# benbergner/ips

Hardware: AMD Instinct MI355X
Metric: patches scored/sec (no-grad IPS loop) (higher is better)
Workload: dtype f32; 1 GPU; Megapixel-MNIST 1500: 2500 patches of 1x32x32 per image (BASELINE configs[1]), B=16, M=64, I=64, n_token=4, use_pos, eager; parallelism=single GPU, dedup_blank=False, patch_storage=f32, loop_workgroups_per_image=1

## Files before the change

### include/ipsx.h

```cpp
#ifndef IPSX_H
#define IPSX_H

#include <stddef.h>
#include <stdint.h>

#ifdef __cplusplus
extern "C" {
#endif

#define IPSX_VERSION 306

#define IPSX_OK            0
#define IPSX_EINVAL       -1
#define IPSX_EHIP         -2
#define IPSX_EWORKSPACE   -3

int ipsx_version(void);
const char* ipsx_last_error(void);
int ipsx_device_count(void);
int ipsx_device_is_gfx950(int dev);


size_t ipsx_packed_conv_weight_elems(int c_out, int c_in, int kh, int kw);

// ... 187 lines not shown
size_t ipsx_projector_stream_ctl_zero_words(int64_t n);
int ipsx_projector_stream_supported(const ipsx_conv* lin, int64_t n, int r);
int ipsx_projector_stats_indexed(const void* x, int dtype, const int32_t* index, int64_t src_rows, int64_t n, int f,
                                 float ln_eps, float* stats, void* stream);
int ipsx_projector_apply_indexed(const ipsx_conv* lin, const float* x, const int32_t* index, int64_t src_rows, int64_t n,
                                 const float* stats, float* out, int32_t* ready, int32_t value, void* stream);
int ipsx_projector_apply_bf16_indexed(const ipsx_conv* lin, const void* x, int dtype, const int32_t* index, int64_t src_rows,
                                      int64_t n, const float* stats, float* out, int32_t* ready, int32_t ready_value,
                                      void* stream);
int ipsx_projector_stream_indexed(const ipsx_conv* lin, const float* x, const int32_t* index, int64_t src_rows, int64_t n,
                                  int64_t slide_rows, float ln_eps, float* emb, const float* v_packed, int r, float* logits,
                                  int32_t* ctl, int32_t* ready, int workgroups, int short_first, void* stream);
int ipsx_projector_stream(const ipsx_conv* lin, const float* x, int64_t n, int64_t slide_rows, float ln_eps, float* emb,
                          const float* v_packed, int r, float* logits, int32_t* ctl, int32_t* ready,
                          int workgroups, int short_first, void* stream);


int ipsx_query_proj(const float* q, const float* wq, float temperature,
                    int n_token, int d, int hdk, float* qs, void* stream);

size_t ipsx_folded_query_elems(int h, int n_token, int d);
int ipsx_fold_query(const float* qs, const float* wk_packed, int h, int dk, int n_token, int d,
                    float* v_packed, void* stream);
int ipsx_logits(const float* emb, int64_t emb_bstride,
                const float* pos, int64_t pos_bstride,
                const float* v_packed,
                int b, int64_t n, int d, int r,
                float* logits, int64_t logits_bstride, void* stream);

int ipsx_logits_if(const float* emb, int64_t emb_bstride, const float* pos, int64_t pos_bstride,
                   const float* v_packed, int b, int64_t n, int d, int r,
                   float* logits, int64_t logits_bstride, const int32_t* cond, int32_t cond_mask, void* stream);

size_t ipsx_folded_query_bf16_bytes(int h, int n_token, int d);
int ipsx_fold_query_bf16(const float* qs, const float* wk_packed, int h, int dk, int n_token, int d,
                         void* v_packed_bf16, void* stream);
int ipsx_logits_bf16(const float* emb, int64_t emb_bstride, const float* pos, int64_t pos_bstride,
                     const void* v_packed_bf16, int b, int64_t n, int d, int r,
                     float* logits, int64_t logits_bstride, void* stream);

int ipsx_set_tie_order(int mode);

int ipsx_scan(const float* logits, int b, int64_t n, int m, int i, int h, int n_token,
              int64_t* mem_idx, float* mem_score, int32_t* tie_flag,
              void* workspace, size_t workspace_bytes, void* stream);

size_t ipsx_scan_workspace_bytes(int b, int m, int i, int h, int n_token);
int ipsx_scan_workgroups_per_image(int b, int m, int i, int h, int n_token);

int ipsx_scan_range(const float* logits, int b, int64_t n, int m, int i, int h, int n_token,
                    int64_t it_begin, int64_t it_end, int64_t* mem_idx, float* mem_score,
                    int32_t* tie_flag, void* workspace, size_t workspace_bytes, void* stream);
int ipsx_scan_range_strided(const float* logits, int64_t logits_bstride_rows, int b, int64_t n, int m, int i, int h,
                            int n_token, int64_t it_begin, int64_t it_end, int64_t* mem_idx, float* mem_score,
                            int32_t* tie_flag, void* workspace, size_t workspace_bytes, void* stream);
int ipsx_scan_ragged(const float* logits, const int64_t* row_offsets, int b, int64_t n_max, int64_t total, int m, int i,
                     int h, int n_token, int64_t* mem_idx, float* mem_score, int32_t* tie_flag, void* workspace,
                     size_t workspace_bytes, void* stream);
int ipsx_scan_ragged_spans(const float* logits, const int64_t* spans, int b, int64_t n_max, int64_t rows_total, int m, int i,
                           int h, int n_token, int64_t* mem_idx, float* mem_score, int32_t* tie_flag, void* workspace,
                           size_t workspace_bytes, void* stream);

int ipsx_scan_persistent_supported(int m, int i, int h, int n_token);
int ipsx_scan_persistent(const float* logits, int b, int64_t n, int m, int i, int h, int n_token,
                         int64_t* mem_idx, float* mem_score, int32_t* tie_flag, const int32_t* ready,
                         int32_t ready_per_image, int32_t* status, void* stream);
int ipsx_scan_persistent_groupable(int m, int i, int h, int n_token);
int ipsx_scan_persistent_on(const float* logits, int b, int64_t n, int m, int i, int h, int n_token,
                            int64_t* mem_idx, float* mem_score, int32_t* tie_flag, const int32_t* ready,
                            int32_t ready_per_image, int32_t* status, int workgroups, void* stream);
int ipsx_scan_persistent_ws(const float* logits, int b, int64_t n, int m, int i, int h, int n_token,
                            int64_t* mem_idx, float* mem_score, int32_t* tie_flag, const int32_t* ready,
                            int32_t ready_per_image, int32_t* status, int workgroups, void* workspace,
                            size_t workspace_bytes, void* stream);
int ipsx_scan_range_if_ws(const float* logits, int b, int64_t n, int m, int i, int h, int n_token,
                          int64_t it_begin, int64_t it_end, int64_t* mem_idx, float* mem_score,
                          int32_t* tie_flag, const int32_t* cond, int32_t cond_mask, void* workspace,
                          size_t workspace_bytes, void* stream);
int ipsx_publish_rows(int32_t* ready, int32_t value, void* stream);
int ipsx_set_persistent_wait_ms(int ms);
int ipsx_scan_range_if(const float* logits, int b, int64_t n, int m, int i, int h, int n_token,
                       int64_t it_begin, int64_t it_end, int64_t* mem_idx, float* mem_score,
                       int32_t* tie_flag, const int32_t* cond, int32_t cond_mask, void* stream);
int ipsx_logits_stats(const float* emb, int64_t emb_bstride, const float* pos, int64_t pos_bstride,
                      const float* v_packed, int b, int64_t n, int d, int r, float* logits, int64_t logits_bstride,
                      const float* stats_x, int64_t stats_n, int stats_f, float ln_eps, float* stats_out, void* stream);
int ipsx_scan_gate(const int32_t* status, void* stream);

int ipsx_scores(const float* x, const float* wk_packed, const float* qs,
                int b, int l, int d, int h, int dk, int n_token,
                float* scores, float* attn, void* workspace, size_t workspace_bytes,
                void* stream);
size_t ipsx_scores_workspace_bytes(int b, int l, int d, int h, int n_token);

int ipsx_topm(const float* scores, int b, int l, int m, int64_t* top_idx,
              int32_t* tie_flag, void* workspace, size_t workspace_bytes, void* stream);
size_t ipsx_topm_workspace_bytes(int b, int l, int m);

int ipsx_gather_rows(const void* src, const int64_t* idx, void* dst,
                     int b, int64_t n_rows, int m, int64_t row_bytes,
                     int64_t src_bstride_rows, void* stream);

int ipsx_ips_finish(const void* patches, int64_t patch_row_bytes, int64_t patch_bstride_rows, int64_t n_rows,
                    const void* pos, int64_t pos_row_bytes, int64_t pos_bstride_rows, const int64_t* mem_idx, int b, int m,
                    void* mem_patch, void* mem_pos, int64_t* mem_idx_out, const int32_t* status, int32_t* status_host,
                    void* stream);
int ipsx_ips_finish_indexed(const void* patches, int64_t patch_row_bytes, int64_t patch_bstride_rows, int64_t n_rows,
                            const void* pos, int64_t pos_row_bytes, int64_t pos_bstride_rows, const int64_t* mem_idx,
                            const int64_t* order, int64_t order_bstride, int b, int m, void* mem_patch, void* mem_pos,
                            int64_t* mem_idx_out, const int32_t* status, int32_t* status_host, void* stream);

int ipsx_ragged_finish(const void* rows, int64_t row_bytes, int64_t total, const int64_t* row_offsets,
                       const int64_t* mem_idx, const int32_t* flat, const void* pos, int64_t pos_row_bytes, int b, int m,
                       void* mem_patch, void* mem_pos, int64_t* mem_idx_out, int64_t* rows_out, void* stream);

typedef struct ipsx_image_entry {
    int64_t elem_off;
    int64_t first;
    int32_t h, w, ny, nx;
} ipsx_image_entry;

typedef struct ipsx_ragged_view {
    int b, c, ph, pw, sh, sw;
    const ipsx_image_entry* images;
    const ipsx_image_entry* host;
} ipsx_ragged_view;

int64_t ipsx_ragged_view_fill(ipsx_image_entry* table, int b, int c, int ph, int pw, int sh, int sw, const int32_t* h,
                              const int32_t* w, const int64_t* elem_off);
int64_t ipsx_ragged_view_offset(const ipsx_image_entry* table, int b, const ipsx_ragged_view* geometry, int64_t p,
                                int64_t* pitch, int64_t* chan_pitch);
int ipsx_trunk_ragged_view_supported(const ipsx_trunk* t, const ipsx_ragged_view* view);
int ipsx_trunk_encode_ragged_view(const ipsx_trunk* t, const float* pixels, const ipsx_ragged_view* view,
                                  const int32_t* index , int64_t first, int64_t n,
                                  float* emb, void* workspace, size_t workspace_bytes, void* stream);
int ipsx_ragged_finish_view(const float* pixels, const ipsx_ragged_view* view, const int64_t* row_offsets, const int64_t* mem_idx,
                            int m, const int32_t* flat, const void* pos, int64_t pos_row_bytes, void* mem_patch, void* mem_pos,
                            int64_t* mem_idx_out, int64_t* rows_out, void* stream);

int ipsx_ragged_view_blank_flags(const float* pixels, const ipsx_ragged_view* view, const int32_t* index,
                                 int64_t first, int64_t n, int32_t* nonblank, void* stream);
size_t ipsx_trunk_ragged_view_dedup_workspace_bytes(const ipsx_trunk* t, int64_t n);
int ipsx_trunk_encode_ragged_view_dedup(const ipsx_trunk* t, const float* pixels, const ipsx_ragged_view* view,
                                        const int32_t* index , int64_t first,
                                        int64_t n, float* emb, void* workspace, size_t workspace_bytes, int32_t* n_encoded,
                                        void* stream);

int ipsx_trunk_encode_ragged_view_u8(const ipsx_trunk* t, const uint8_t* pixels, const float* table, const ipsx_ragged_view* view,
                                     const int32_t* index , int64_t first, int64_t n,
                                     float* emb, void* workspace, size_t workspace_bytes, void* stream);
int ipsx_ragged_finish_view_u8(const uint8_t* pixels, const float* table, const ipsx_ragged_view* view, const int64_t* row_offsets,
                               const int64_t* mem_idx, int m, const int32_t* flat, const void* pos, int64_t pos_row_bytes,
                               void* mem_patch, void* mem_pos, int64_t* mem_idx_out, int64_t* rows_out, void* stream);
int ipsx_ragged_view_blank_flags_u8(const uint8_t* pixels, const ipsx_ragged_view* view, const int32_t* index, int64_t first,
                                    int64_t n, int32_t* nonblank, void* stream);
int ipsx_trunk_encode_ragged_view_dedup_u8(const ipsx_trunk* t, const uint8_t* pixels, const float* table,
                                           const ipsx_ragged_view* view, const int32_t* index, int64_t first, int64_t n, float* emb,
                                           void* workspace, size_t workspace_bytes, int32_t* n_encoded, void* stream);

typedef struct ipsx_stream_table {
    const void* held;
    int64_t held_rows, held_bstride_rows;
    const void* piece;
    int64_t piece_bstride_bytes;
    void* dst;
    int64_t dst_rows, dst_bstride_rows;
// ... 91 lines not shown
```

### ips_amd/architecture/ips_net.py

```python

import contextlib
import os

import torch
from torch import nn

from .. import hip
from ..ragged import Ragged
from ..ragged_image import RaggedImages
from ..shuffle import draw_shuffle, shuffle_batch, shuffle_instance
from .resnet import load_torchvision_checkpoint, resnet18_trunk, resnet50_trunk
from .transformer import Transformer, pos_enc_1d


class IPSNet(nn.Module):

    def get_conv_patch_enc(self, enc_type, pretrained, n_chan_in, n_res_blocks):
        if enc_type == 'resnet18':
            trunk = resnet18_trunk()
        elif enc_type == 'resnet50':
            trunk = resnet50_trunk()
        else:
            raise ValueError("unknown enc_type {!r}".format(enc_type))
        if pretrained:
# ... 156 lines not shown
            if fused:
                preds[task['name']] = hip.head(embeddings, task['id'], layer[0], task['act_fn'])
            else:
                preds[task['name']] = layer(embeddings[:, task['id']])
        return preds

    def _embed(self, x):
        if hip.on_device(x) and not self.encoder.training and not (
                torch.is_grad_enabled() and any(p.requires_grad for p in self.encoder.parameters())):
            return self.plan.encode(x, table=self._table_for(x))
        if x.dtype == torch.uint8:
            x = self._dequant(x)
        if hip.on_device(x) and self.encoder.training and self.is_image and torch.is_grad_enabled():
            from ..training import fused_encoder
            if getattr(self, "_fused_train_ok", None) is None:
                self._fused_train_ok = fused_encoder.supported(self.encoder)
            if self._fused_train_ok and fused_encoder.enabled():
                return fused_encoder.encode(self.encoder, x)
        if hip.on_device(x) and self.encoder.training and not self.is_image and torch.is_grad_enabled():
            from ..training import fused_projector
            if getattr(self, "_fused_train_ok", None) is None:
                self._fused_train_ok = fused_projector.supported(self.encoder)
            if self._fused_train_ok and fused_projector.enabled() and x.dim() == 2 and x.shape[0] > 1 and not x.requires_grad:
                return fused_projector.encode(self.encoder, x)
        if not self.is_image and x.dtype in (torch.float16, torch.bfloat16):
            x = x.float()
        return self.encoder(x).flatten(1)

    @torch.no_grad()
    def ips(self, patches):
        if isinstance(patches, Ragged):
            return self.ips_ragged(patches, pad=patches.pad)
        B, N = patches.shape[:2]
        u8 = patches.dtype == torch.uint8
        if u8:
            self._check_u8(patches)
        if self.M >= N:
            self._reset_last()
            mem_patch = patches.to(self.device)
            return (self._dequant(mem_patch) if u8 else mem_patch), (self.pos_enc.expand(B, -1, -1) if self.use_pos else None)
        return self._call(patches)

    @torch.no_grad()
    def ips_ragged(self, slides, pad=False):
        from ..ragged import ips_ragged
        return ips_ragged(self, slides, pad)

    def _reset_last(self):
        self.last_mem_idx = None
        self.last_shuffle = None
        self._emb_parts = None
        self._mem_emb = None
        self._emb_make = None
        self._mem_count = None

    @contextlib.contextmanager
    def _scoring(self):
        was_training = self.training
        if was_training:
            self.encoder.eval()
            self.transf.eval()
        try:
            yield
        finally:
            if was_training:
                self.encoder.train()
                self.transf.train()

    def _call(self, patches):
        device, pos_enc = self.device, self.pos_enc
        viewed = not torch.is_tensor(patches)
        u8 = patches.dtype == torch.uint8
        B = patches.shape[0]
        self._reset_last()
        with self._scoring():
            if self.use_pos:
                pos_enc = pos_enc.expand(B, -1, -1)
            order = None
            if self.shuffle:
                patches, pos_enc, order = self._shuffle(patches, pos_enc)

            if hip.on_device(device):
                with self.plan.hold():
                    mem_idx = self._select_hip(patches, pos_enc, order)
            else:
                mem_idx = self._select_aten(patches, pos_enc)

            src = self._device_patches if self._device_patches is not None else patches
            self._device_patches = None
            sel = self._selection
            done = sel.finish(src, pos_enc if self.use_pos else None, order) if sel is not None else None
            if done is not None:
                mem_idx, mem_patch, mem_pos = done
            else:
                if sel is not None:
                    mem_idx = sel.take_unfinished(mem_idx)
                rows = mem_idx if order is None else torch.gather(order.expand(B, -1), 1, mem_idx)
                if viewed:
                    mem_patch = hip.gather_patches_view(src.images, src.view, rows, self._table_for(src))
                else:
                    mem_patch = self._take(src, rows).to(device)
                mem_pos = self._take(pos_enc, mem_idx) if self.use_pos else None
                if sel is not None:
                    sel.after_call()
            if u8 and not viewed:
                mem_patch = self._dequant(mem_patch)

        self.last_mem_idx = mem_idx
        return mem_patch, mem_pos

    @staticmethod
    def _unfold_images(images, patch_size, patch_stride):
        (ph, pw), (sh, sw) = patch_size, patch_stride
        if ph > images.shape[2] or pw > images.shape[3] or min(ph, pw, sh, sw) <= 0:
            raise ValueError("patch {}x{} / stride {}x{} does not fit a {}x{} image".format(ph, pw, sh, sw, *images.shape[2:]))
        p = images.unfold(2, ph, sh).unfold(3, pw, sw).permute(0, 2, 3, 1, 4, 5)
        return p.reshape(images.shape[0], -1, images.shape[1], ph, pw)

    def _materialise(self, images, patch_size, patch_stride):
        if hip.on_device(self.device):
            images = images.to(self.device)
            if images.dtype == torch.float32:
                return hip.patchify(images, patch_size, patch_stride)
        return self._unfold_images(images, patch_size, patch_stride).contiguous()

    @torch.no_grad()
    def ips_image(self, images, patch_size, patch_stride):
        if isinstance(images, RaggedImages):
            return self.ips_image_ragged(images, patch_size, patch_stride, pad=images.pad)
        if not self.is_image or images.dim() != 4:
            raise TypeError("ips_image takes (B, C, H, W) images of an image encoder")
        table = self._table_for(images)
        view = None
        if (hip.on_device(self.device) and images.dtype in (torch.float32, torch.uint8) and not hip.dedup_blank()
                and not (self.encoder.training and not self.training)
                and not (self.shuffle and self._shuffle_overridden())):
            view = hip.PatchView(images.shape, patch_size, patch_stride)
            if self.M >= view.per_image or not self.plan.view_supported(view):
                view = None
        if view is None:
            return self.ips(self._materialise(images, patch_size, patch_stride))
        return self._call(hip.PatchSource(images=images.to(self.device), view=view, table=table))

    @torch.no_grad()
    def ips_image_ragged(self, images, patch_size, patch_stride, pad=False):
        from ..ragged_image import ips_image_ragged
        return ips_image_ragged(self, images, patch_size, patch_stride, pad)

    def ips_stream(self, patch_size=None, patch_stride=None):
        from ..stream import IPSStream
        return IPSStream(self, patch_size, patch_stride)

    def ips_ragged_stream(self, pad=False, patch_size=None, patch_stride=None):
        from ..ragged_stream import RaggedIPSStream
        return RaggedIPSStream(self, pad, patch_size, patch_stride)

    def _chunks(self, N):
        yield 0, self.M
        for start in range(self.M, N, self.I):
            yield start, min(start + self.I, N)

    @staticmethod
    def _take(src, idx):
        if hip.on_device(src):
            return hip.gather_rows(src, idx)
        idx = idx.to(src.device)
        view = idx.view(*idx.shape, *(1,) * (src.dim() - 2)).expand(-1, -1, *src.shape[2:])
# ... 67 lines not shown
```

### ips_amd/csrc/logits.hip

```cpp

#include <algorithm>
#include <cstdlib>

#include "scan_common.h"

namespace ipsx {

__global__ void query_proj_kernel(const float* __restrict__ q, const float* __restrict__ wq, float temperature,
                                  int n_token, int d, int hdk, float* __restrict__ qs) {
    const int i = blockIdx.x * blockDim.x + threadIdx.x;
    if (i >= n_token * hdk) return;
    const int t = i / hdk, o = i - t * hdk;
    float a = 0.0f;
    for (int c = 0; c < d; ++c) a = __builtin_fmaf(q[t * d + c], wq[(size_t)o * d + c], a);
    qs[i] = a / temperature;
}

__global__ void fold_query_kernel(const float* __restrict__ qs, const float* __restrict__ wkp, int h, int dk, int T, int d,
                                  int kgs, int r_pad, float* __restrict__ vp) {
    const int idx = blockIdx.x * blockDim.x + threadIdx.x;
    const int dpad = kgs * 8;
    if (idx >= r_pad * dpad) return;
    const int r = idx / dpad, c = idx - r * dpad;
    const int R = h * T, hdk = h * dk;
    float acc = 0.0f;
    if (r < R && c < d) {
        const int hh = r / T, t = r - hh * T;
        const int kg = c >> 3, sub = c & 7;
        for (int j = 0; j < dk; ++j) {
            const int o = hh * dk + j;
            const float w = wkp[(((size_t)(o >> 5) * kgs + kg) * 64 + (o & 31) + 32 * (sub >> 2)) * 4 + (sub & 3)];
            acc = __builtin_fmaf(qs[(size_t)t * hdk + o], w, acc);
        }
    }
    vp[(((size_t)(r >> 5) * kgs + (c >> 3)) * 64 + (r & 31) + 32 * ((c & 7) >> 2)) * 4 + (c & 3)] = acc;
}

struct LogitsArgs {
    const float* emb; long long emb_bs;
    const float* pos; long long pos_bs;
    const float* vp;
    long long n;
    int d, R, kgs;
    float* out; long long out_bs;
};

template <int NT>
__device__ __forceinline__ void logits_wave(const LogitsArgs& a, unsigned bx, int bi) {
    const int lane = threadIdx.x & 63, wave = threadIdx.x >> 6, half = lane >> 5;
    const long long r0 = ((long long)bx * 4 + wave) * 32;
    if (r0 >= a.n) return;
    const long long row = r0 + (lane & 31);
    const bool rv = row < a.n;
    const float* e = a.emb + (size_t)bi * a.emb_bs + (size_t)(rv ? row : 0) * a.d + 4 * half;
    const float* p = a.pos ? a.pos + (size_t)bi * a.pos_bs + (size_t)(rv ? row : 0) * a.d + 4 * half : nullptr;

    f32x16 acc[NT];
#pragma unroll
    for (int i = 0; i < NT; ++i)
#pragma unroll
        for (int r = 0; r < 16; ++r) acc[i][r] = 0.0f;

    const float4* vq = reinterpret_cast<const float4*>(a.vp) + lane;
    const bool vec = (a.d & 7) == 0;
    int kg0 = 0;
    if (vec) {
        float4 ev[2][8], bv[2][NT][8];
        auto fetch = [&](int k0, int set) {
#pragma unroll
            for (int u = 0; u < 8; ++u) {
                ev[set][u] = *reinterpret_cast<const float4*>(e + (k0 + u) * 8);
                if (p) {
                    const float4 pv = *reinterpret_cast<const float4*>(p + (k0 + u) * 8);
                    ev[set][u].x = ev[set][u].x + pv.x; ev[set][u].y = ev[set][u].y + pv.y;
                    ev[set][u].z = ev[set][u].z + pv.z; ev[set][u].w = ev[set][u].w + pv.w;
                }
#pragma unroll
                for (int i = 0; i < NT; ++i) bv[set][i][u] = vq[((size_t)i * a.kgs + k0 + u) * 64];
            }
        };
        auto mma = [&](int set) {
#pragma unroll
            for (int u = 0; u < 8; ++u) {
                const float a0 = rv ? ev[set][u].x : 0.0f, a1 = rv ? ev[set][u].y : 0.0f;
                const float a2 = rv ? ev[set][u].z : 0.0f, a3 = rv ? ev[set][u].w : 0.0f;
#pragma unroll
                for (int i = 0; i < NT; ++i) {
                    acc[i] = __builtin_amdgcn_mfma_f32_32x32x2f32(a0, bv[set][i][u].x, acc[i], 0, 0, 0);
                    acc[i] = __builtin_amdgcn_mfma_f32_32x32x2f32(a1, bv[set][i][u].y, acc[i], 0, 0, 0);
                    acc[i] = __builtin_amdgcn_mfma_f32_32x32x2f32(a2, bv[set][i][u].z, acc[i], 0, 0, 0);
                    acc[i] = __builtin_amdgcn_mfma_f32_32x32x2f32(a3, bv[set][i][u].w, acc[i], 0, 0, 0);
                }
            }
        };
        if (a.kgs >= 8) {
            fetch(0, 0);
            for (; kg0 + 16 <= a.kgs; kg0 += 16) {
                fetch(kg0 + 8, 1);
                mma(0);
                if (kg0 + 24 <= a.kgs) fetch(kg0 + 16, 0);
                mma(1);
            }
            if (kg0 + 8 <= a.kgs) { mma(0); kg0 += 8; }
        }
    }
    for (int kg = kg0; kg < a.kgs; ++kg) {
        float av[4];
        if (vec) {
            const float4 ev = *reinterpret_cast<const float4*>(e + kg * 8);
            av[0] = ev.x; av[1] = ev.y; av[2] = ev.z; av[3] = ev.w;
            if (p) {
                const float4 pv = *reinterpret_cast<const float4*>(p + kg * 8);
                av[0] = av[0] + pv.x; av[1] = av[1] + pv.y; av[2] = av[2] + pv.z; av[3] = av[3] + pv.w;
            }
#pragma unroll
            for (int j = 0; j < 4; ++j) av[j] = rv ? av[j] : 0.0f;
        } else {
#pragma unroll
            for (int j = 0; j < 4; ++j) {
                const int c = kg * 8 + j;
                float v = (c + 4 * half < a.d) ? e[c] : 0.0f;
                if (p) v = v + ((c + 4 * half < a.d) ? p[c] : 0.0f);
                av[j] = rv ? v : 0.0f;
            }
        }
#pragma unroll
        for (int i = 0; i < NT; ++i) {
            const float4 b = vq[((size_t)i * a.kgs + kg) * 64];
            acc[i] = __builtin_amdgcn_mfma_f32_32x32x2f32(av[0], b.x, acc[i], 0, 0, 0);
            acc[i] = __builtin_amdgcn_mfma_f32_32x32x2f32(av[1], b.y, acc[i], 0, 0, 0);
            acc[i] = __builtin_amdgcn_mfma_f32_32x32x2f32(av[2], b.z, acc[i], 0, 0, 0);
            acc[i] = __builtin_amdgcn_mfma_f32_32x32x2f32(av[3], b.w, acc[i], 0, 0, 0);
        }
    }
    float* out = a.out + (size_t)bi * a.out_bs;
#pragma unroll
    for (int i = 0; i < NT; ++i) {
        const int o = i * 32 + (lane & 31);
        if (o < a.R) {
#pragma unroll
            for (int r = 0; r < 16; ++r) {
                const long long rr = r0 + (r & 3) + 8 * (r >> 2) + 4 * half;
                if (rr < a.n) out[(size_t)rr * a.R + o] = acc[i][r];
            }
        }
    }
}

template <int NT>
__global__ __launch_bounds__(256) void logits_kernel(LogitsArgs a) { logits_wave<NT>(a, blockIdx.x, (int)blockIdx.y); }

template <int NT>
__global__ __launch_bounds__(256) void logits_if_kernel(LogitsArgs a, const int* cond, int mask) {
    if ((__hip_atomic_load(cond, __ATOMIC_RELAXED, __HIP_MEMORY_SCOPE_AGENT) & mask) == 0) return;
    logits_wave<NT>(a, blockIdx.x, (int)blockIdx.y);
}

template <int NT>
__global__ __launch_bounds__(256) void logits_stats_kernel(LogitsArgs a, unsigned n_logits_x, const float* __restrict__ sx,
                                                           long long sn, int sf, float eps, float2* __restrict__ sout) {
    if (blockIdx.x < n_logits_x) { logits_wave<NT>(a, blockIdx.x, (int)blockIdx.y); return; }
    if (blockIdx.y != 0) return;
    const int lane = threadIdx.x & 63;
    const long long row0 = ((long long)(blockIdx.x - n_logits_x) * 4 + (threadIdx.x >> 6)) * 32;
    if (row0 >= sn) return;
    const float2 st = row_moments_wave32(sx, row0, sn, sf, eps, lane);
    if (lane < 32 && row0 + lane < sn) sout[row0 + lane] = st;
}

typedef __bf16 bf16x8_t __attribute__((ext_vector_type(8)));

__global__ void fold_query_bf16_kernel(const float* __restrict__ qs, const float* __restrict__ wkp, int h, int dk, int T, int d,
                                       int kgs, int ksteps, int r_pad, unsigned short* __restrict__ vq16) {
    const int idx = blockIdx.x * blockDim.x + threadIdx.x;
    const int dpad = ksteps * 16;
    if (idx >= r_pad * dpad) return;
    const int r = idx / dpad, c = idx - r * dpad;
    const int R = h * T, hdk = h * dk;
    float acc = 0.0f;
    if (r < R && c < d) {
        const int hh = r / T, t = r - hh * T;
        const int kg = c >> 3, sub = c & 7;
        for (int j = 0; j < dk; ++j) {
            const int o = hh * dk + j;
            const float w = wkp[(((size_t)(o >> 5) * kgs + kg) * 64 + (o & 31) + 32 * (sub >> 2)) * 4 + (sub & 3)];
            acc = __builtin_fmaf(qs[(size_t)t * hdk + o], w, acc);
        }
    }
    const __bf16 hv = (__bf16)acc;
    vq16[(((size_t)(r >> 5) * ksteps + (c >> 4)) * 64 + (r & 31) + 32 * ((c & 15) >> 3)) * 8 + (c & 7)] =
        __builtin_bit_cast(unsigned short, hv);
}

template <int NT>
__global__ __launch_bounds__(256) void logits_bf16_kernel(LogitsArgs a, const uint4* __restrict__ vq16, int ksteps) {
    const int lane = threadIdx.x & 63, wave = threadIdx.x >> 6, half = lane >> 5;
    const long long r0 = ((long long)blockIdx.x * 4 + wave) * 32;
    if (r0 >= a.n) return;
    const int bi = blockIdx.y;
    const long long row = r0 + (lane & 31);
    const bool rv = row < a.n;
    const float* e = a.emb + (size_t)bi * a.emb_bs + (size_t)(rv ? row : 0) * a.d + 8 * half;
    const float* p = a.pos ? a.pos + (size_t)bi * a.pos_bs + (size_t)(rv ? row : 0) * a.d + 8 * half : nullptr;
    f32x16 acc[NT];
#pragma unroll
    for (int i = 0; i < NT; ++i)
#pragma unroll
        for (int r = 0; r < 16; ++r) acc[i][r] = 0.0f;
    for (int ks = 0; ks < ksteps; ++ks) {
        float xv[8];
#pragma unroll
        for (int j = 0; j < 8; ++j) {
            const int c = ks * 16 + 8 * half + j;
            float v = (rv && c < a.d) ? e[ks * 16 + j] : 0.0f;
            if (p) v = v + ((rv && c < a.d) ? p[ks * 16 + j] : 0.0f);
            xv[j] = v;
        }
        bf16x8_t av;
#pragma unroll
        for (int j = 0; j < 8; ++j) av[j] = (__bf16)xv[j];
#pragma unroll
        for (int i = 0; i < NT; ++i) {
            const uint4 b = vq16[((size_t)i * ksteps + ks) * 64 + lane];
            acc[i] = __builtin_amdgcn_mfma_f32_32x32x16_bf16(av, __builtin_bit_cast(bf16x8_t, b), acc[i], 0, 0, 0);
        }
    }
    float* out = a.out + (size_t)bi * a.out_bs;
#pragma unroll
    for (int i = 0; i < NT; ++i) {
// ... 147 lines not shown
```

### ips_amd/csrc/scan_common.h

```cpp
#pragma once

#include <algorithm>
#include <cstdlib>
#include <type_traits>

#include "ipsx_common.h"
#include "ipsx_math.h"
#include "ipsx_rowstats.h"
#include "ipsx_stdorder.h"

namespace ipsx {

typedef float f32x16 __attribute__((ext_vector_type(16)));

struct CandView {
    const float* cl;
    const float* lg;
    const int* cand;
    int R;
    __device__ __forceinline__ float get(int l, int r) const {
        if (cl) return cl[l * (R + 1) + r];
        const size_t row = cand ? (size_t)cand[l] : (size_t)l;
        return lg[row * R + r];
    }
// ... 822 lines not shown
                while (v_ >= 0 && v_ < (need)) {                                                               \
                    __builtin_amdgcn_s_sleep(16);                                                              \
                    int w_ = lane < a.ready_words ? __hip_atomic_load(a.ready + lane, __ATOMIC_RELAXED, __HIP_MEMORY_SCOPE_AGENT) : 0; \
                    for (int o_ = 32; o_ >= 1; o_ >>= 1) w_ += __shfl_xor(w_, o_, 64);                         \
                    const unsigned long long now_ = __builtin_amdgcn_s_memrealtime();                          \
                    if (w_ != seen_) { seen_ = w_; t0_ = now_; }                                               \
                    if (now_ - t0_ > a.wait_ticks) { v_ = -1; break; }                                         \
                    v_ = __hip_atomic_load(a.ready + b * a.ready_stride, __ATOMIC_RELAXED, __HIP_MEMORY_SCOPE_AGENT); \
                }                                                                                              \
                if (lane == 0) ccount[6] = v_;                                                     \
            }                                                                                                  \
            lds_barrier();                                                                                     \
             \
             \
            __builtin_amdgcn_fence(__ATOMIC_ACQUIRE, "agent");                                                 \
            ready_known = ccount[6];                                                               \
            if (ready_known < 0) {                                                                             \
                if (tid == 0) { __hip_atomic_fetch_or(a.status, 1, __ATOMIC_RELAXED, __HIP_MEMORY_SCOPE_AGENT); a.plog[5] += 1; } \
                return;                                                                                        \
            }                                                                                                  \
        }                                                                                                      \
    } while (0)

template <int N, int J>
__device__ __forceinline__ uint32_t cmpx32(uint32_t s, uint32_t dir, int lane) {
    const uint32_t o = lane_xor_u32<J>(s, lane);
    const uint32_t c = (uint32_t)__builtin_amdgcn_sbfe((int)dir, N, 1);
    uint32_t d;
    asm("v_med3_u32 %0, %1, %2, %3" : "=v"(d) : "v"(s), "v"(o), "v"(c));
    return d;
}

__device__ __forceinline__ uint32_t sort_directions(int lane) {
    constexpr int KJ[21][2] = {{2, 1}, {4, 2}, {4, 1}, {8, 4}, {8, 2}, {8, 1}, {16, 8}, {16, 4}, {16, 2}, {16, 1}, {32, 16}, {32, 8},
                               {32, 4}, {32, 2}, {32, 1}, {64, 32}, {64, 16}, {64, 8}, {64, 4}, {64, 2}, {64, 1}};
    uint32_t d = 0u;
#pragma unroll
    for (int n = 0; n < 21; ++n) d |= ((((lane & KJ[n][0]) == 0) == ((lane & KJ[n][1]) == 0)) ? 1u : 0u) << n;
    return d;
}

__device__ __forceinline__ uint32_t wave_sort_desc_u32(uint32_t s, uint32_t dir, int lane) {
    s = cmpx32<0, 1>(s, dir, lane);
    s = cmpx32<1, 2>(s, dir, lane); s = cmpx32<2, 1>(s, dir, lane);
    s = cmpx32<3, 4>(s, dir, lane); s = cmpx32<4, 2>(s, dir, lane); s = cmpx32<5, 1>(s, dir, lane);
    s = cmpx32<6, 8>(s, dir, lane); s = cmpx32<7, 4>(s, dir, lane); s = cmpx32<8, 2>(s, dir, lane); s = cmpx32<9, 1>(s, dir, lane);
    s = cmpx32<10, 16>(s, dir, lane); s = cmpx32<11, 8>(s, dir, lane); s = cmpx32<12, 4>(s, dir, lane); s = cmpx32<13, 2>(s, dir, lane);
    s = cmpx32<14, 1>(s, dir, lane);
    s = cmpx32<15, 32>(s, dir, lane); s = cmpx32<16, 16>(s, dir, lane); s = cmpx32<17, 8>(s, dir, lane); s = cmpx32<18, 4>(s, dir, lane);
    s = cmpx32<19, 2>(s, dir, lane); s = cmpx32<20, 1>(s, dir, lane);
    return s;
}

struct TopmArgs {
    int tie_order, stk_off;
    const float* scores;
    int L, m, n2;
    long long* top;
    int* tie;
};

struct ScanCall {
    const float* logits = nullptr;
    int b = 0;
    int64_t n = 0;
    int m = 0, i = 0, h = 0, n_token = 0;
    int64_t it_begin = 0, it_end = 0;
    int64_t* mem_idx = nullptr;
    float* mem_score = nullptr;
    int32_t* tie_flag = nullptr;
    const int32_t* ready = nullptr;
    int32_t* status = nullptr;
    void* workspace = nullptr;
    size_t workspace_bytes = 0;
    void* stream = nullptr;
    const int32_t* cond = nullptr;
    int32_t cond_mask = 0;
    int ready_stride = 0, workgroups = 0;
    Rows rows = Rows::Packed;
    const int64_t* slide_table = nullptr;
    int64_t table_rows = 0;
};

inline const long long* slide_entries(const ScanCall& c) {
    static_assert(sizeof(long long) == sizeof(int64_t), "slide tables: 64-bit entries");
    return static_cast<const long long*>(static_cast<const void*>(c.slide_table));
}

struct FastPlan {
    bool ok;
    int ept, lch;
    size_t lds;
};
FastPlan scan_fast_plan(int m, int i, int h, int n_token);
int launch_scan_fast(const ScanCall& c, const FastPlan& fp);
bool scan_cam_shape(int m, int i, int h, int n_token);
int launch_scan_cam(const ScanCall& c);
bool scan_mnist_shape(int m, int i, int h, int n_token);
int launch_scan_mnist(const ScanCall& c);
size_t scan_large_ws_per_image(int m, int i, int h, int n_token);
int launch_scan_large(const ScanCall& c);
int scan_large_team(int b, int m, int i, int h, int n_token);
int launch_topm_large(const TopmArgs& a, int b, void* workspace, size_t workspace_bytes, void* stream);
size_t topm_large_ws_per_row(int l);
int scan_large_max_l();

extern int g_persist_wait_ms;
extern bool g_scan_generic;
extern bool g_replay_stamps_on;
extern bool g_scan_direct;
extern bool g_scan_team_trunc;
extern int g_scan_team;
extern bool g_scan_r8;
extern bool g_scan_mnist;
extern unsigned long long* g_scan_stamps;
unsigned long long* persist_log();

inline int next_pow2(int v) { int p = 1; while (p < v) p <<= 1; return p; }
constexpr size_t kLdsLimit = 160 * 1024;

inline void fill_scan_args(ScanArgs& a, const ScanCall& c) {
    a.plog = persist_log();
    a.lg = c.logits; a.n = c.n; a.table_rows = c.table_rows; a.m = c.m; a.i = c.i; a.h = c.h; a.T = c.n_token; a.n2 = next_pow2(c.m + c.i);
    a.it0 = c.it_begin; a.it1 = c.it_end;
    a.mem_idx = reinterpret_cast<long long*>(c.mem_idx); a.mem_score = c.mem_score; a.tie = c.tie_flag;
    a.ready = c.ready; a.status = c.status; a.ready_stride = c.ready_stride;
    a.ready_words = c.ready ? (c.ready_stride ? std::min(c.b, 64) : 1) : 0;
    a.wait_ticks = (unsigned long long)g_persist_wait_ms * 100000ull;
    a.cond = c.cond; a.cond_mask = c.cond_mask;
    a.slides = c.b;
    a.tie_order = g_tie_order;
    a.use_lds = 1;
    a.stk_off = 0;
}

template <typename T> struct as_declared { using type = T; };
template <typename... A>
inline void launch_lds(void (*kernel)(A...), dim3 grid, dim3 block, size_t lds, void* stream, typename as_declared<A>::type... args) {
    (void)hipFuncSetAttribute(reinterpret_cast<const void*>(kernel), hipFuncAttributeMaxDynamicSharedMemorySize, (int)lds);
    kernel<<<grid, block, lds, as_stream(stream)>>>(args...);
}

}
```

### ips_amd/csrc/scan_mnist.hip

```cpp

#include <algorithm>
#include <cstdlib>

#include "scan_common.h"

namespace ipsx {

namespace mn {
constexpr int M = 64, I = 64, L = 128, R = 32, H = 8, T = 4, LD = 36, NT = 1024;
constexpr int OFF_KEYA = 0;
constexpr int OFF_SORTED = OFF_KEYA + L * 8;
constexpr int OFF_CAND = OFF_SORTED + L * 8;
constexpr int OFF_PMAX = OFF_CAND + 2 * L * 4;
constexpr int OFF_CNT = OFF_PMAX + 4 * R * 4;
constexpr int OFF_PREV = OFF_CNT + 32;
constexpr int OFF_DEN = OFF_PREV + 2 * R * 4;
constexpr int OFF_X = (OFF_DEN + R * 4 + 15) & ~15;
constexpr int OFF_E = OFF_X + 2 * L * LD * 4;
constexpr int OFF_STK = OFF_E + 2 * L * LD * 4;
constexpr int LDS_BYTES = OFF_STK + STK_BYTES;
static_assert(OFF_KEYA % 16 == 0 && OFF_X % 16 == 0 && (LD * 4) % 16 == 0, "16-byte rows");
static_assert(H * T == R && M + I == L && L * 8 == NT, "scan_mnist_kernel: 8 threads per key");
static_assert(OFF_STK == 77728, "scan_mnist_kernel: 77,728 B of LDS + the replay's scratch (STK_BYTES)");
static_assert(LDS_BYTES <= 160 * 1024, "scan_mnist_kernel: LDS");
}

template <int K>
__device__ __forceinline__ float quad_bcast(float v) {
    return as_float((uint32_t)__builtin_amdgcn_update_dpp(0, (int)as_u32(v), K * 0x55, 0xF, 0xF, false));
}

template <bool PERSIST>
__global__ __launch_bounds__(mn::NT) void scan_mnist_kernel(ScanArgs a) {
    using namespace mn;
    extern __shared__ __attribute__((aligned(16))) unsigned char smem[];
    if (!PERSIST && scan_skipped(a.cond, a.cond_mask)) return;
    __builtin_amdgcn_s_setprio(3);
    if (PERSIST) {
        asm volatile("v_mov_b32 v127, 0" ::: "v127");
        if (threadIdx.x == 0) {
            __hip_atomic_fetch_or(a.status, 2, __ATOMIC_RELAXED, __HIP_MEMORY_SCOPE_AGENT);
            __hip_atomic_store(&a.plog[4], (unsigned long long)__builtin_amdgcn_s_memrealtime(), __ATOMIC_RELAXED, __HIP_MEMORY_SCOPE_AGENT);
        }
    }
    uint64_t* const keyA = reinterpret_cast<uint64_t*>(smem + OFF_KEYA);
    uint64_t* const sorted = reinterpret_cast<uint64_t*>(smem + OFF_SORTED);
    uint32_t* const pmax = reinterpret_cast<uint32_t*>(smem + OFF_PMAX);
    int* const ccount = reinterpret_cast<int*>(smem + OFF_CNT);
    uint32_t* const prevk = reinterpret_cast<uint32_t*>(smem + OFF_PREV);
    float* const rden = reinterpret_cast<float*>(smem + OFF_DEN);
    const int tid = threadIdx.x, lane = tid & 63, wave = tid >> 6;
    const int b = blockIdx.x;
    const int r = tid & (R - 1);
    const int hid = tid - 512;
    const float* const lg = a.lg + (size_t)b * a.n * R;
    int ready_known = 0;
    if (tid < 4 * R) pmax[tid] = 0u;
    if (tid < 2) ccount[2 + tid] = 0;
    lds_barrier();
    SCAN_WAIT_ROWS(std::min<long long>(a.n, a.it0 * (long long)I + M + I));
    {
        float* const x0 = reinterpret_cast<float*>(smem + OFF_X);
        int* const cand0 = reinterpret_cast<int*>(smem + OFF_CAND);
        uint32_t km = 0u;
#pragma unroll
        for (int k = 0; k < 2; ++k) {
            const int l = (tid >> 5) + 32 * k;
            const size_t row = a.it0 == 0 ? (size_t)l : (size_t)a.mem_idx[(size_t)b * M + l];
            const float v = scan_load<PERSIST>(lg + row * R + r);
            x0[l * LD + r] = v;
            km = max(km, max_key(v));
        }
        fold_row_max<R>(km, pmax, lane);
        if (tid < M) cand0[tid] = a.it0 == 0 ? tid : (int)a.mem_idx[(size_t)b * M + tid];
    }
    const long long n_iter = a.it1 - a.it0;
    float pf[4];
    {
        float* const x0 = reinterpret_cast<float*>(smem + OFF_X);
        int* const cand0 = reinterpret_cast<int*>(smem + OFF_CAND);
        const long long lo = a.it0 * (long long)I + M;
        const int cnt = n_iter > 0 ? (int)std::min<long long>(I, a.n - lo) : 0;
        uint32_t kc = 0u;
#pragma unroll
        for (int k = 0; k < 2; ++k) {
            const int e = tid + NT * k;
            if (e < cnt * R) {
                const float v = scan_load<PERSIST>(lg + (size_t)lo * R + e);
                x0[(M + (e >> 5)) * LD + r] = v;
                kc = max(kc, max_key(v));
            }
        }
        fold_row_max<R>(kc, pmax + R, lane);
        if (tid < cnt) cand0[M + tid] = (int)(lo + tid);
        const long long lo1 = lo + I;
        const int cnt1 = n_iter > 1 ? (int)std::max<long long>(0, std::min<long long>(I, a.n - lo1)) : 0;
        if (cnt1 > 0) SCAN_WAIT_ROWS(lo1 + cnt1);
#pragma unroll
        for (int k = 0; k < 4; ++k) {
            const int e = hid + 512 * k;
            pf[k] = (hid >= 0 && e < cnt1 * R) ? scan_load<PERSIST>(lg + (size_t)lo1 * R + e) : 0.0f;
        }
    }
    int tie = 0;
    const int n_it = (int)n_iter, n_rows = (int)a.n;
    for (int k_it = 0; k_it < n_it; ++k_it) {
        const int lo = ((int)a.it0 + k_it) * I + M;
        const int cnt = min(I, n_rows - lo);
        const int Lc = M + cnt;
        const int par = k_it & 1;
        float* const xc = reinterpret_cast<float*>(smem + OFF_X) + par * (L * LD);
        float* const xn = reinterpret_cast<float*>(smem + OFF_X) + (par ^ 1) * (L * LD);
        float* const ec = reinterpret_cast<float*>(smem + OFF_E) + par * (L * LD);
        float* const en = reinterpret_cast<float*>(smem + OFF_E) + (par ^ 1) * (L * LD);
        int* const cand = reinterpret_cast<int*>(smem + OFF_CAND) + par * L;
        int* const cnew = reinterpret_cast<int*>(smem + OFF_CAND) + (par ^ 1) * L;
        uint32_t* const mkey = pmax + 2 * R * par;
        uint32_t* const mkey_nx = pmax + 2 * R * (par ^ 1);
        const int lo1 = lo + I;
        const int cnt1 = k_it + 1 < n_it ? max(0, min(I, n_rows - lo1)) : 0;
        lds_barrier();
        if (tid == 0) ccount[2 + (par ^ 1)] = 0;
        const uint32_t mbits = as_u32(max_key_value(max(mkey[r], mkey[R + r])));
        const float rowmax = as_float(mbits);
        const bool changed = k_it == 0 || prevk[par * R + r] != mbits;
        if (tid < R) prevk[(par ^ 1) * R + r] = mbits;
        {
            unsigned long long moved = __ballot(changed) & 0xFFFFFFFFull;
            if (moved != 0ull) {
                if (__popcll(moved) >= 8) {
                    if (changed) {
#pragma unroll
                        for (int k = 0; k < 4; ++k) {
                            const int l = (tid >> 5) + 32 * k;
                            if (l < Lc) ec[l * LD + r] = det_expf_np(xc[l * LD + r] - rowmax);
                        }
                    }
                } else {
                    while (moved) {
                        const int rr = __ffsll((long long)moved) - 1;
                        moved &= moved - 1ull;
                        exp_column(xc + rr, ec + rr, Lc, LD, __shfl(rowmax, rr, 64));
// ... 62 lines not shown
            const uint32_t* const sw = reinterpret_cast<const uint32_t*>(sorted);
            const unsigned long long eqm = __ballot(sw[2 * lane + 1] == sw[2 * lane + 3]);
            if (eqm != 0ull) {
                if (a.tie_order != 0) {
                    bool hit = false;
                    for (int j = tid; j < M && !hit; j += NT)
                        for (int k = j + 1; k < Lc && !hit && (sorted[k] >> 32) == (sorted[j] >> 32); ++k) {
                            bool same = true;
                            if (a.tie_order == 1) {
                                const uint4* ra = reinterpret_cast<const uint4*>(xc + key_pos(sorted[j]) * LD);
                                const uint4* rb = reinterpret_cast<const uint4*>(xc + key_pos(sorted[k]) * LD);
                                uint32_t diff = 0u;
#pragma unroll
                                for (int rr = 0; rr < R / 4; ++rr) {
                                    const uint4 va = ra[rr], vb = rb[rr];
                                    diff |= (va.x ^ vb.x) | (va.y ^ vb.y) | (va.z ^ vb.z) | (va.w ^ vb.w);
                                }
                                same = diff == 0u;
                            }
                            hit = hit || same;
                        }
                    if (__ballot(hit) != 0ull && lane == 0) ccount[2 + par] = 1;
                }
                lds_barrier();
                if (tid == 0 && (eqm >> (M - 1)) != 0ull) tie = 1;
                if (a.tie_order != 0 && ccount[2 + par] != 0)
                    tie_order_slow(sorted, keyA, Lc, M, reinterpret_cast<int*>(smem + OFF_STK));
            }
        }
        {
            const int lo2 = lo + 2 * I;
            const int cnt2 = k_it + 2 < n_it ? max(0, min(I, n_rows - lo2)) : 0;
            if (cnt2 > 0) SCAN_WAIT_ROWS(lo2 + cnt2);
#pragma unroll
            for (int k = 0; k < 4; ++k) {
                const int e = hid + 512 * k;
                pf[k] = (hid >= 0 && e < cnt2 * R) ? scan_load<PERSIST>(lg + (size_t)lo2 * R + e) : 0.0f;
            }
        }
        {
            const uint32_t* const spos = reinterpret_cast<const uint32_t*>(sorted);
            if (wave < 8) {
                uint32_t p[4];
#pragma unroll
                for (int k = 0; k < 4; ++k) p[k] = ~spos[2 * ((tid >> 5) + 16 * k)] & (L - 1);
                float gx[4];
#pragma unroll
                for (int k = 0; k < 4; ++k) gx[k] = xc[p[k] * LD + r];
                uint32_t km = 0u;
#pragma unroll
                for (int k = 0; k < 4; ++k) { xn[((tid >> 5) + 16 * k) * LD + r] = gx[k]; km = max(km, max_key(gx[k])); }
                fold_row_max<R>(km, mkey_nx, lane);
            } else {
                const int j = hid >> 3, qd = (hid & 7) * 4;
                const uint32_t p = ~spos[2 * j] & (L - 1);
                const uint32_t pc = ~spos[2 * (hid & (M - 1))] & (L - 1);
                const float4 ge = *reinterpret_cast<const float4*>(ec + p * LD + qd);
                const int ci = cand[pc];
                *reinterpret_cast<float4*>(en + j * LD + qd) = ge;
                if (hid < M) cnew[hid] = ci;
            }
        }
    }
    lds_barrier();
    {
        const int parn = (int)(n_iter & 1);
        const int* const cand = reinterpret_cast<const int*>(smem + OFF_CAND) + parn * L;
        if (tid < M) {
            a.mem_idx[(size_t)b * M + tid] = cand[tid];
            if (a.mem_score) a.mem_score[(size_t)b * M + tid] = n_iter > 0 ? key_score(sorted[tid]) : 0.0f;
        }
    }
    if (a.tie && tid == 0 && tie) a.tie[b] = 1;
}

bool scan_mnist_shape(int m, int i, int h, int n_token) { return h == mn::H && n_token == mn::T && m == mn::M && i == mn::I; }

int launch_scan_mnist(const ScanCall& c) {
    IPSX_REQUIRE(scan_mnist_shape(c.m, c.i, c.h, c.n_token) && c.rows == Rows::Packed && (c.workgroups <= 0 || c.workgroups >= c.b),
                 "scan_mnist_kernel: 8 heads x 4 tokens, M = I = 64, contiguous logits, one workgroup per image");
    ScanArgs a;
    fill_scan_args(a, c);
    a.stk_off = mn::OFF_STK;
    launch_lds(c.ready ? scan_mnist_kernel<true> : scan_mnist_kernel<false>, dim3((unsigned)c.b), dim3(mn::NT), mn::LDS_BYTES, c.stream, a);
    return launched("scan");
}

}
```

### ips_amd/csrc/scorer.hip

```cpp

#include <algorithm>
#include <cstdlib>

#include "scan_common.h"

namespace ipsx {

int g_tie_order = 1;
int g_persist_wait_ms = 50;
bool g_scan_generic = false;
bool g_replay_stamps_on = false;
bool g_scan_team_trunc = true;
int g_scan_team = -1;
bool g_scan_direct = true;
bool g_scan_r8 = true;
bool g_scan_mnist = true;
unsigned long long* g_scan_stamps = nullptr;

__device__ unsigned long long g_persist_log[8];


unsigned long long* persist_log() {
    static unsigned long long* p[64] = {nullptr};
    int dev = 0;
    if (hipGetDevice(&dev) != hipSuccess || dev < 0 || dev >= 64) dev = 0;
    if (!p[dev]) {
        void* q = nullptr;
        if (hipGetSymbolAddress(&q, HIP_SYMBOL(g_persist_log)) == hipSuccess) p[dev] = static_cast<unsigned long long*>(q);
    }
    return p[dev];
}

static ScanCall scan_call(const float* logits, int b, int64_t n, int m, int i, int h, int n_token, int64_t* mem_idx,
                          float* mem_score, int32_t* tie_flag, void* stream) {
    ScanCall c;
    c.logits = logits; c.b = b; c.n = n; c.m = m; c.i = i; c.h = h; c.n_token = n_token;
    c.mem_idx = mem_idx; c.mem_score = mem_score; c.tie_flag = tie_flag; c.stream = stream;
    return c;
}

static void whole_loop(ScanCall& c) { c.it_begin = 0; c.it_end = (c.n - c.m + c.i - 1) / c.i; }

static int validate_scan_call(const ScanCall& c) {
    IPSX_REQUIRE(c.logits && c.mem_idx, "scan: null pointer");
    IPSX_REQUIRE(c.b > 0 && c.m > 0 && c.i > 0 && c.h > 0 && c.n_token > 0, "scan: bad sizes");
    IPSX_REQUIRE(c.n > c.m, "scan: needs more patches (%lld) than memory slots (%d)", (long long)c.n, c.m);
    IPSX_REQUIRE(c.n < ((int64_t)1 << 31), "scan: too many patches");
    IPSX_REQUIRE(c.it_begin >= 0 && c.it_begin <= c.it_end && c.it_end <= (c.n - c.m + c.i - 1) / c.i,
                 "scan: iteration range [%lld, %lld) outside the loop", (long long)c.it_begin, (long long)c.it_end);
    if (c.rows == Rows::Packed) return IPSX_OK;
    IPSX_REQUIRE(!c.ready && !c.cond && !g_scan_stamps,
                 "scan: only packed logits are waited for (persistent), launched conditionally or stamped");
    IPSX_REQUIRE(c.table_rows > 0 && c.table_rows < ((int64_t)1 << 31), "scan: a table of %lld rows", (long long)c.table_rows);
    if (rows_per_slide(c.rows)) {
        IPSX_REQUIRE(c.slide_table, "scan: slides without their table");
        IPSX_REQUIRE(c.workgroups <= 0 || c.workgroups >= c.b, "scan: slides of different lengths take a workgroup each");
    }
    return IPSX_OK;
}

static int dispatch_scan(const ScanCall& c) {
    IPSX_TRY(validate_scan_call(c));
    if (c.it_begin == c.it_end) return IPSX_OK;
    const FastPlan fp = scan_fast_plan(c.m, c.i, c.h, c.n_token);
    if (!fp.ok || (g_scan_generic && !c.ready && !c.cond)) return launch_scan_large(c);
    if (g_scan_r8 && scan_cam_shape(c.m, c.i, c.h, c.n_token)) return launch_scan_cam(c);
    if (g_scan_mnist && scan_mnist_shape(c.m, c.i, c.h, c.n_token) && c.rows == Rows::Packed &&
        (c.workgroups <= 0 || c.workgroups >= c.b) && g_scan_stamps == nullptr)
        return launch_scan_mnist(c);
    return launch_scan_fast(c, fp);
}

}

using namespace ipsx;

IPSX_API int ipsx_scan(const float* logits, int b, int64_t n, int m, int i, int h, int n_token,
                       int64_t* mem_idx, float* mem_score, int32_t* tie_flag, void* workspace, size_t workspace_bytes,
                       void* stream) {
    IPSX_REQUIRE(n > m && i > 0, "scan: needs more patches (%lld) than memory slots (%d)", (long long)n, m);
    if (tie_flag && hipMemsetAsync(tie_flag, 0, sizeof(int32_t) * (size_t)std::max(b, 0), as_stream(stream)) != hipSuccess)
        return fail(IPSX_EHIP, "scan: memset failed");
    return ipsx_scan_range(logits, b, n, m, i, h, n_token, 0, (n - m + i - 1) / i, mem_idx, mem_score, tie_flag,
                           workspace, workspace_bytes, stream);
}

IPSX_API int ipsx_scan_range(const float* logits, int b, int64_t n, int m, int i, int h, int n_token,
                             int64_t it_begin, int64_t it_end, int64_t* mem_idx, float* mem_score,
                             int32_t* tie_flag, void* workspace, size_t workspace_bytes, void* stream) {
    ScanCall c = scan_call(logits, b, n, m, i, h, n_token, mem_idx, mem_score, tie_flag, stream);
    c.it_begin = it_begin; c.it_end = it_end;
    c.workspace = workspace; c.workspace_bytes = workspace_bytes;
    return dispatch_scan(c);
}

IPSX_API int ipsx_scan_range_strided(const float* logits, int64_t logits_bstride_rows, int b, int64_t n, int m, int i, int h,
                                     int n_token, int64_t it_begin, int64_t it_end, int64_t* mem_idx, float* mem_score,
                                     int32_t* tie_flag, void* workspace, size_t workspace_bytes, void* stream) {
    IPSX_REQUIRE(logits_bstride_rows >= n && logits_bstride_rows < ((int64_t)1 << 31),
// ... 101 lines not shown
    whole_loop(c);
    c.ready = ready; c.ready_stride = ready_per_image ? 1 : 0; c.status = status;
    c.workgroups = workgroups;
    c.workspace = workspace; c.workspace_bytes = workspace_bytes;
    return dispatch_scan(c);
}

IPSX_API int ipsx_scan_range_if_ws(const float* logits, int b, int64_t n, int m, int i, int h, int n_token,
                                   int64_t it_begin, int64_t it_end, int64_t* mem_idx, float* mem_score,
                                   int32_t* tie_flag, const int32_t* cond, int32_t cond_mask, void* workspace,
                                   size_t workspace_bytes, void* stream) {
    IPSX_REQUIRE(cond && cond_mask, "scan_range_if: needs the condition word and a mask");
    ScanCall c = scan_call(logits, b, n, m, i, h, n_token, mem_idx, mem_score, tie_flag, stream);
    c.it_begin = it_begin; c.it_end = it_end;
    c.cond = cond; c.cond_mask = cond_mask;
    c.workspace = workspace; c.workspace_bytes = workspace_bytes;
    return dispatch_scan(c);
}

__global__ void scan_gate_kernel(const int* status, unsigned long long wait_ticks) {
    const unsigned long long t0 = __builtin_amdgcn_s_memrealtime();
    bool gave_up = false;
    while ((__hip_atomic_load(status, __ATOMIC_RELAXED, __HIP_MEMORY_SCOPE_AGENT) & 2) == 0) {
        __builtin_amdgcn_s_sleep(8);
        if (__builtin_amdgcn_s_memrealtime() - t0 > wait_ticks) { gave_up = true; break; }
    }
    const unsigned long long waited = __builtin_amdgcn_s_memrealtime() - t0;
    g_persist_log[0] += 1;
    g_persist_log[3] = t0;
    if (gave_up) g_persist_log[2] += 1;
    if (waited > g_persist_log[1]) {
        g_persist_log[1] = waited;
        g_persist_log[6] = t0;
        g_persist_log[7] = gave_up ? 0ull : __hip_atomic_load(&g_persist_log[4], __ATOMIC_RELAXED, __HIP_MEMORY_SCOPE_AGENT);
    }
}

IPSX_API int ipsx_scan_gate(const int32_t* status, void* stream) {
    IPSX_REQUIRE(status, "scan_gate: null pointer");
    scan_gate_kernel<<<dim3(1), dim3(1), 0, as_stream(stream)>>>(status, (unsigned long long)g_persist_wait_ms * 100000ull);
    return launched("scan_gate");
}

__global__ void part_wait_kernel(const int* done, int want, int* status, int bit, unsigned long long wait_ticks) {
    unsigned long long t0 = __builtin_amdgcn_s_memrealtime();
    int last = __hip_atomic_load(done, __ATOMIC_RELAXED, __HIP_MEMORY_SCOPE_AGENT);
    while (last < want) {
        __builtin_amdgcn_s_sleep(32);
        const int v = __hip_atomic_load(done, __ATOMIC_RELAXED, __HIP_MEMORY_SCOPE_AGENT);
        const unsigned long long t = __builtin_amdgcn_s_memrealtime();
        if (v != last) { last = v; t0 = t; }
        else if (t - t0 > wait_ticks) {
            __hip_atomic_fetch_or(status, bit, __ATOMIC_RELAXED, __HIP_MEMORY_SCOPE_AGENT);
            break;
        }
    }
    __builtin_amdgcn_fence(__ATOMIC_ACQUIRE, "agent");
}

IPSX_API int ipsx_part_wait(const int32_t* done, int32_t want, int32_t* status, int32_t bit, void* stream) {
    IPSX_REQUIRE(done && status && bit, "part_wait: needs the counter, the status word and a bit");
    part_wait_kernel<<<dim3(1), dim3(1), 0, as_stream(stream)>>>(done, want, status, bit,
                                                                 (unsigned long long)g_persist_wait_ms * 100000ull);
    return launched("part_wait");
}

IPSX_API int ipsx_publish_rows(int32_t* ready, int32_t value, void* stream) {
    IPSX_REQUIRE(ready, "publish_rows: null pointer");
    publish_rows_kernel<<<dim3(1), dim3(1), 0, as_stream(stream)>>>(ready, value);
    return launched("publish_rows");
}

IPSX_API int ipsx_scan_range_if(const float* logits, int b, int64_t n, int m, int i, int h, int n_token,
                                int64_t it_begin, int64_t it_end, int64_t* mem_idx, float* mem_score,
                                int32_t* tie_flag, const int32_t* cond, int32_t cond_mask, void* stream) {
    IPSX_REQUIRE(cond && cond_mask, "scan_range_if: needs the condition word and a mask");
    IPSX_REQUIRE(scan_fast_plan(m, i, h, n_token).ok, "scan_range_if: shapes of the LDS-resident loop only");
    ScanCall c = scan_call(logits, b, n, m, i, h, n_token, mem_idx, mem_score, tie_flag, stream);
    c.it_begin = it_begin; c.it_end = it_end;
    c.cond = cond; c.cond_mask = cond_mask;
    return dispatch_scan(c);
}

IPSX_API int ipsx_set_persistent_wait_ms(int ms) {
    const int prev = g_persist_wait_ms;
    if (ms > 0) g_persist_wait_ms = ms > 20000 ? 20000 : ms;
    return prev;
}

IPSX_API int ipsx_set_tie_order(int mode) {
    const int prev = ipsx::g_tie_order;
    if (mode >= 0 && mode <= 2) ipsx::g_tie_order = mode;
    return prev;
}

extern "C" __attribute__((visibility("default"))) int ipsx_dbg_persist_log(unsigned long long* out8) {
    unsigned long long zero[8] = {0, 0, 0, 0, 0, 0, 0, 0};
    if (hipMemcpyFromSymbol(out8, HIP_SYMBOL(ipsx::g_persist_log), sizeof(zero)) != hipSuccess) return -1;
    return hipMemcpyToSymbol(HIP_SYMBOL(ipsx::g_persist_log), zero, sizeof(zero)) == hipSuccess ? 0 : -1;
}

extern "C" __attribute__((visibility("default"))) void ipsx_dbg_scan_stamps(unsigned long long* buf) {
    ipsx::g_scan_stamps = buf;
}

extern "C" __attribute__((visibility("default"))) void ipsx_dbg_scan_generic(int on) { g_scan_generic = on != 0; }

extern "C" __attribute__((visibility("default"))) void ipsx_dbg_scan_direct(int on) { g_scan_direct = on != 0; }
extern "C" __attribute__((visibility("default"))) void ipsx_dbg_scan_team(int w) { g_scan_team = w; }
extern "C" __attribute__((visibility("default"))) void ipsx_dbg_scan_team_trunc(int on) { g_scan_team_trunc = on != 0; }
extern "C" __attribute__((visibility("default"))) void ipsx_dbg_scan_r8(int on) { g_scan_r8 = on != 0; }
extern "C" __attribute__((visibility("default"))) void ipsx_dbg_scan_mnist(int on) { g_scan_mnist = on != 0; }
extern "C" __attribute__((visibility("default"))) int ipsx_dbg_scan_mnist_shape(int m, int i, int h, int n_token) {
    return scan_mnist_shape(m, i, h, n_token) ? 1 : 0;
}
```

### ips_amd/hip.py

```python

import collections
import ctypes as C
import os
import subprocess

import torch

_PKG = os.path.dirname(os.path.abspath(__file__))
_SO = os.path.join(_PKG, "lib", "libipsx.so")
_LIB = None

f32p = C.c_void_p
ABI_MAJOR = 3


def backend():
    b = os.environ.get("IPSX_BACKEND", "hip").lower()
    if b not in ("hip", "aten"):
        raise ValueError("IPSX_BACKEND must be 'hip' or 'aten', got {!r}".format(b))
    return b


def precision():
    p = os.environ.get("IPSX_PRECISION", "fp32").lower()
# ... 223 lines not shown
    "ipsx_projector_stats_indexed": (C.c_int, [C.c_void_p, C.c_int, C.c_void_p, C.c_int64, C.c_int64, C.c_int, C.c_float, C.c_void_p,
                                               C.c_void_p]),
    "ipsx_projector_apply_indexed": (C.c_int, [C.POINTER(Conv), C.c_void_p, C.c_void_p, C.c_int64, C.c_int64, C.c_void_p, C.c_void_p,
                                               C.c_void_p, C.c_int32, C.c_void_p]),
    "ipsx_projector_apply_bf16_indexed": (C.c_int, [C.POINTER(Conv), C.c_void_p, C.c_int, C.c_void_p, C.c_int64, C.c_int64, C.c_void_p,
                                                    C.c_void_p, C.c_void_p, C.c_int32, C.c_void_p]),
    "ipsx_projector_stream_indexed": (C.c_int, [C.POINTER(Conv), C.c_void_p, C.c_void_p, C.c_int64, C.c_int64, C.c_int64, C.c_float,
                                                C.c_void_p, C.c_void_p, C.c_int, C.c_void_p, C.c_void_p, C.c_void_p, C.c_int, C.c_int,
                                                C.c_void_p]),
    "ipsx_trunk_stream_ctl_words": (C.c_size_t, [C.c_int64]),
    "ipsx_trunk_stream_supported": (C.c_int, [C.POINTER(Trunk), C.c_int, C.c_int]),
    "ipsx_trunk_stream": (C.c_int, [C.POINTER(Trunk), C.c_void_p, C.c_int64, C.c_void_p, C.c_void_p, C.c_void_p, C.c_int,
                                    C.c_void_p, C.c_void_p, C.c_void_p, C.c_int, C.c_int, C.c_void_p]),
    "ipsx_projector_stream_ctl_words": (C.c_size_t, [C.c_int64]),
    "ipsx_projector_stream_ctl_zero_words": (C.c_size_t, [C.c_int64]),
    "ipsx_projector_stream_supported": (C.c_int, [C.POINTER(Conv), C.c_int64, C.c_int]),
    "ipsx_projector_stream": (C.c_int, [C.POINTER(Conv), C.c_void_p, C.c_int64, C.c_int64, C.c_float, C.c_void_p, C.c_void_p, C.c_int,
                                        C.c_void_p, C.c_void_p, C.c_void_p, C.c_int, C.c_int, C.c_void_p]),
    "ipsx_logits_stats": (C.c_int, [C.c_void_p, C.c_int64, C.c_void_p, C.c_int64, C.c_void_p,
                                    C.c_int, C.c_int64, C.c_int, C.c_int, C.c_void_p, C.c_int64,
                                    C.c_void_p, C.c_int64, C.c_int, C.c_float, C.c_void_p, C.c_void_p]),
    "ipsx_query_proj": (C.c_int, [C.c_void_p, C.c_void_p, C.c_float, C.c_int, C.c_int, C.c_int,
                                  C.c_void_p, C.c_void_p]),
    "ipsx_folded_query_elems": (C.c_size_t, [C.c_int, C.c_int, C.c_int]),
    "ipsx_fold_query": (C.c_int, [C.c_void_p, C.c_void_p, C.c_int, C.c_int, C.c_int, C.c_int, C.c_void_p, C.c_void_p]),
    "ipsx_logits": (C.c_int, [C.c_void_p, C.c_int64, C.c_void_p, C.c_int64, C.c_void_p,
                              C.c_int, C.c_int64, C.c_int, C.c_int,
                              C.c_void_p, C.c_int64, C.c_void_p]),
    "ipsx_folded_query_bf16_bytes": (C.c_size_t, [C.c_int, C.c_int, C.c_int]),
    "ipsx_fold_query_bf16": (C.c_int, [C.c_void_p, C.c_void_p, C.c_int, C.c_int, C.c_int, C.c_int, C.c_void_p, C.c_void_p]),
    "ipsx_logits_bf16": (C.c_int, [C.c_void_p, C.c_int64, C.c_void_p, C.c_int64, C.c_void_p,
                                   C.c_int, C.c_int64, C.c_int, C.c_int,
                                   C.c_void_p, C.c_int64, C.c_void_p]),
    "ipsx_set_tie_order": (C.c_int, [C.c_int]),
    "ipsx_scan": (C.c_int, [C.c_void_p, C.c_int, C.c_int64, C.c_int, C.c_int, C.c_int, C.c_int,
                            C.c_void_p, C.c_void_p, C.c_void_p, C.c_void_p, C.c_size_t, C.c_void_p]),
    "ipsx_scan_workspace_bytes": (C.c_size_t, [C.c_int] * 5),
    "ipsx_scan_workgroups_per_image": (C.c_int, [C.c_int] * 5),
    "ipsx_scan_range": (C.c_int, [C.c_void_p, C.c_int, C.c_int64, C.c_int, C.c_int, C.c_int, C.c_int, C.c_int64, C.c_int64,
                                  C.c_void_p, C.c_void_p, C.c_void_p, C.c_void_p, C.c_size_t, C.c_void_p]),
    "ipsx_scan_range_strided": (C.c_int, [C.c_void_p, C.c_int64, C.c_int, C.c_int64, C.c_int, C.c_int, C.c_int, C.c_int, C.c_int64,
                                          C.c_int64, C.c_void_p, C.c_void_p, C.c_void_p, C.c_void_p, C.c_size_t, C.c_void_p]),
    "ipsx_scan_ragged": (C.c_int, [C.c_void_p, C.c_void_p, C.c_int, C.c_int64, C.c_int64, C.c_int, C.c_int, C.c_int, C.c_int,
                                   C.c_void_p, C.c_void_p, C.c_void_p, C.c_void_p, C.c_size_t, C.c_void_p]),
    "ipsx_stream_commit": (C.c_int, [C.POINTER(StreamTable), C.c_int, C.c_void_p, C.c_int, C.c_int, C.c_int64, C.c_int64,
                                     C.c_void_p]),
    "ipsx_stream_commit_view": (C.c_int, [C.POINTER(StreamTable), C.c_int, C.c_void_p, C.POINTER(PatchViewStruct), C.c_int,
                                          C.c_void_p, C.c_int, C.c_int, C.c_int64, C.c_int64, C.POINTER(C.c_int), C.c_void_p]),
    "ipsx_scan_range_if": (C.c_int, [C.c_void_p, C.c_int, C.c_int64, C.c_int, C.c_int, C.c_int, C.c_int, C.c_int64, C.c_int64,
                                     C.c_void_p, C.c_void_p, C.c_void_p, C.c_void_p, C.c_int32, C.c_void_p]),
    "ipsx_scan_persistent_supported": (C.c_int, [C.c_int] * 4),
    "ipsx_scan_persistent_groupable": (C.c_int, [C.c_int] * 4),
    "ipsx_scan_persistent_on": (C.c_int, [C.c_void_p, C.c_int, C.c_int64, C.c_int, C.c_int, C.c_int, C.c_int,
                                          C.c_void_p, C.c_void_p, C.c_void_p, C.c_void_p, C.c_int32, C.c_void_p, C.c_int,
                                          C.c_void_p]),
    "ipsx_scan_persistent_ws": (C.c_int, [C.c_void_p, C.c_int, C.c_int64, C.c_int, C.c_int, C.c_int, C.c_int,
                                          C.c_void_p, C.c_void_p, C.c_void_p, C.c_void_p, C.c_int32, C.c_void_p, C.c_int,
                                          C.c_void_p, C.c_size_t, C.c_void_p]),
    "ipsx_scan_range_if_ws": (C.c_int, [C.c_void_p, C.c_int, C.c_int64, C.c_int, C.c_int, C.c_int, C.c_int, C.c_int64, C.c_int64,
                                        C.c_void_p, C.c_void_p, C.c_void_p, C.c_void_p, C.c_int32, C.c_void_p, C.c_size_t,
                                        C.c_void_p]),
    "ipsx_scan_persistent": (C.c_int, [C.c_void_p, C.c_int, C.c_int64, C.c_int, C.c_int, C.c_int, C.c_int,
                                       C.c_void_p, C.c_void_p, C.c_void_p, C.c_void_p, C.c_int32, C.c_void_p, C.c_void_p]),
    "ipsx_publish_rows": (C.c_int, [C.c_void_p, C.c_int32, C.c_void_p]),
    "ipsx_set_persistent_wait_ms": (C.c_int, [C.c_int]),
    "ipsx_scan_gate": (C.c_int, [C.c_void_p, C.c_void_p]),
    "ipsx_trunk_encode_indexed": (C.c_int, [C.POINTER(Trunk), C.c_void_p, C.c_void_p, C.c_int64, C.c_void_p, C.c_void_p]),
    "ipsx_trunk_encode_parts": (C.c_int, [C.POINTER(Trunk), C.c_void_p, C.c_void_p, C.c_int64, C.c_void_p,
                                          C.POINTER(C.c_int64), C.c_int, C.c_void_p, C.c_void_p]),
    "ipsx_trunk_parts_dedup_workspace_bytes": (C.c_size_t, [C.POINTER(Trunk), C.c_int64]),
    "ipsx_trunk_encode_parts_dedup": (C.c_int, [C.POINTER(Trunk), C.c_void_p, C.c_void_p, C.c_int64, C.c_void_p,
                                                C.POINTER(C.c_int64), C.c_int, C.c_void_p, C.c_void_p, C.c_void_p, C.c_size_t,
                                                C.c_void_p, C.c_void_p]),
    "ipsx_trunk_encode_parts_dedup_u8": (C.c_int, [C.POINTER(Trunk), C.c_void_p, C.c_void_p, C.c_void_p, C.c_int64, C.c_void_p,
                                                   C.POINTER(C.c_int64), C.c_int, C.c_void_p, C.c_void_p, C.c_void_p, C.c_size_t,
                                                   C.c_void_p, C.c_void_p]),
    "ipsx_trunk_encode_parts_dedup_view": (C.c_int, [C.POINTER(Trunk), C.c_void_p, C.POINTER(PatchViewStruct), C.c_void_p, C.c_int64,
                                                     C.c_void_p, C.POINTER(C.c_int64), C.c_int, C.c_void_p, C.c_void_p, C.c_void_p,
                                                     C.c_size_t, C.c_void_p, C.c_void_p]),
    "ipsx_trunk_encode_parts_dedup_view_u8": (C.c_int, [C.POINTER(Trunk), C.c_void_p, C.c_void_p, C.POINTER(PatchViewStruct),
                                                        C.c_void_p, C.c_int64, C.c_void_p, C.POINTER(C.c_int64), C.c_int, C.c_void_p,
                                                        C.c_void_p, C.c_void_p, C.c_size_t, C.c_void_p, C.c_void_p]),
    "ipsx_part_wait": (C.c_int, [C.c_void_p, C.c_int32, C.c_void_p, C.c_int32, C.c_void_p]),
    "ipsx_logits_if": (C.c_int, [C.c_void_p, C.c_int64, C.c_void_p, C.c_int64, C.c_void_p, C.c_int, C.c_int64, C.c_int, C.c_int,
                                 C.c_void_p, C.c_int64, C.c_void_p, C.c_int32, C.c_void_p]),
    "ipsx_trunk_encode_u8": (C.c_int, [C.POINTER(Trunk), C.c_void_p, C.c_void_p, C.c_int64, C.c_void_p, C.c_void_p,
                                       C.c_size_t, C.c_void_p]),
    "ipsx_trunk_encode_indexed_u8": (C.c_int, [C.POINTER(Trunk), C.c_void_p, C.c_void_p, C.c_void_p, C.c_int64, C.c_void_p,
                                               C.c_void_p]),
    "ipsx_dequant_patches": (C.c_int, [C.c_void_p, C.c_void_p, C.c_void_p, C.c_int64, C.c_int, C.c_int, C.c_void_p]),
    "ipsx_scores_workspace_bytes": (C.c_size_t, [C.c_int] * 5),
    "ipsx_scores": (C.c_int, [C.c_void_p, C.c_void_p, C.c_void_p] + [C.c_int] * 6 +
                    [C.c_void_p, C.c_void_p, C.c_void_p, C.c_size_t, C.c_void_p]),
    "ipsx_topm": (C.c_int, [C.c_void_p, C.c_int, C.c_int, C.c_int, C.c_void_p, C.c_void_p, C.c_void_p, C.c_size_t, C.c_void_p]),
    "ipsx_topm_workspace_bytes": (C.c_size_t, [C.c_int] * 3),
    "ipsx_gather_rows": (C.c_int, [C.c_void_p, C.c_void_p, C.c_void_p, C.c_int, C.c_int64, C.c_int,
                                   C.c_int64, C.c_int64, C.c_void_p]),
    "ipsx_ips_call_run": (C.c_int, [C.POINTER(IpsCall)]),
    "ipsx_ips_call_elapsed": (C.c_int, [C.c_int, C.POINTER(C.c_float)]),
    "ipsx_ips_call_run_ordered": (C.c_int, [C.POINTER(IpsCall), C.POINTER(IpsCallOrder)]),
    "ipsx_order_index": (C.c_int, [C.c_void_p, C.c_int64, C.c_int, C.c_int64, C.c_void_p, C.c_void_p]),
    "ipsx_trunk_stream_indexed": (C.c_int, [C.POINTER(Trunk), C.c_void_p, C.c_void_p, C.c_int64, C.c_int64, C.c_void_p, C.c_void_p,
                                            C.c_void_p, C.c_int, C.c_void_p, C.c_void_p, C.c_void_p, C.c_int, C.c_int, C.c_void_p]),
    "ipsx_ips_finish": (C.c_int, [C.c_void_p, C.c_int64, C.c_int64, C.c_int64, C.c_void_p, C.c_int64, C.c_int64, C.c_void_p, C.c_int,
                                  C.c_int, C.c_void_p, C.c_void_p, C.c_void_p, C.c_void_p, C.c_void_p, C.c_void_p]),
    "ipsx_ips_finish_indexed": (C.c_int, [C.c_void_p, C.c_int64, C.c_int64, C.c_int64, C.c_void_p, C.c_int64, C.c_int64, C.c_void_p,
                                          C.c_void_p, C.c_int64, C.c_int, C.c_int, C.c_void_p, C.c_void_p, C.c_void_p, C.c_void_p,
                                          C.c_void_p, C.c_void_p]),
    "ipsx_ragged_finish": (C.c_int, [C.c_void_p, C.c_int64, C.c_int64, C.c_void_p, C.c_void_p, C.c_void_p, C.c_void_p, C.c_int64,
                                     C.c_int, C.c_int, C.c_void_p, C.c_void_p, C.c_void_p, C.c_void_p, C.c_void_p]),
    "ipsx_ragged_view_fill": (C.c_int64, [C.POINTER(ImageEntry)] + [C.c_int] * 6 + [C.POINTER(C.c_int32), C.POINTER(C.c_int32),
                                          C.POINTER(C.c_int64)]),
    "ipsx_ragged_view_offset": (C.c_int64, [C.POINTER(ImageEntry), C.c_int, C.POINTER(RaggedViewStruct), C.c_int64,
                                            C.POINTER(C.c_int64), C.POINTER(C.c_int64)]),
    "ipsx_trunk_ragged_view_supported": (C.c_int, [C.POINTER(Trunk), C.POINTER(RaggedViewStruct)]),
    "ipsx_trunk_encode_ragged_view": (C.c_int, [C.POINTER(Trunk), C.c_void_p, C.POINTER(RaggedViewStruct), C.c_void_p, C.c_int64,
                                                C.c_int64, C.c_void_p, C.c_void_p, C.c_size_t, C.c_void_p]),
    "ipsx_ragged_finish_view": (C.c_int, [C.c_void_p, C.POINTER(RaggedViewStruct), C.c_void_p, C.c_void_p, C.c_int, C.c_void_p,
                                          C.c_void_p, C.c_int64, C.c_void_p, C.c_void_p, C.c_void_p, C.c_void_p, C.c_void_p]),
    "ipsx_ragged_view_blank_flags": (C.c_int, [C.c_void_p, C.POINTER(RaggedViewStruct), C.c_void_p, C.c_int64, C.c_int64, C.c_void_p,
                                               C.c_void_p]),
    "ipsx_trunk_ragged_view_dedup_workspace_bytes": (C.c_size_t, [C.POINTER(Trunk), C.c_int64]),
    "ipsx_trunk_encode_ragged_view_dedup": (C.c_int, [C.POINTER(Trunk), C.c_void_p, C.POINTER(RaggedViewStruct), C.c_void_p, C.c_int64,
                                                      C.c_int64, C.c_void_p, C.c_void_p, C.c_size_t, C.c_void_p, C.c_void_p]),
    "ipsx_trunk_encode_ragged_view_u8": (C.c_int, [C.POINTER(Trunk), C.c_void_p, C.c_void_p, C.POINTER(RaggedViewStruct), C.c_void_p,
                                                   C.c_int64, C.c_int64, C.c_void_p, C.c_void_p, C.c_size_t, C.c_void_p]),
    "ipsx_ragged_finish_view_u8": (C.c_int, [C.c_void_p, C.c_void_p, C.POINTER(RaggedViewStruct), C.c_void_p, C.c_void_p, C.c_int,
                                             C.c_void_p, C.c_void_p, C.c_int64, C.c_void_p, C.c_void_p, C.c_void_p, C.c_void_p,
                                             C.c_void_p]),
    "ipsx_ragged_view_blank_flags_u8": (C.c_int, [C.c_void_p, C.POINTER(RaggedViewStruct), C.c_void_p, C.c_int64, C.c_int64,
                                                  C.c_void_p, C.c_void_p]),
    "ipsx_trunk_encode_ragged_view_dedup_u8": (C.c_int, [C.POINTER(Trunk), C.c_void_p, C.c_void_p, C.POINTER(RaggedViewStruct),
                                                         C.c_void_p, C.c_int64, C.c_int64, C.c_void_p, C.c_void_p, C.c_size_t,
                                                         C.c_void_p, C.c_void_p]),
    "ipsx_scan_ragged_spans": (C.c_int, [C.c_void_p, C.c_void_p, C.c_int, C.c_int64, C.c_int64, C.c_int, C.c_int, C.c_int, C.c_int,
                                         C.c_void_p, C.c_void_p, C.c_void_p, C.c_void_p, C.c_size_t, C.c_void_p]),
    "ipsx_stream_commit_ragged": (C.c_int, [C.POINTER(StreamTable), C.c_int, C.c_void_p, C.c_void_p, C.c_int, C.c_int, C.c_int64,
                                            C.c_int64, C.c_void_p]),
    "ipsx_stream_commit_ragged_view": (C.c_int, [C.POINTER(StreamTable), C.c_int, C.c_void_p, C.POINTER(RaggedViewStruct), C.c_int,
                                                 C.c_void_p, C.c_void_p, C.c_int, C.c_int, C.c_int64, C.c_int64, C.POINTER(C.c_int),
                                                 C.c_void_p]),
    "ipsx_aggregate_workspace_bytes": (C.c_size_t, [C.POINTER(Transf), C.c_int, C.c_int]),
    "ipsx_aggregate": (C.c_int, [C.POINTER(Transf), C.c_void_p, C.c_int, C.c_int, C.c_void_p,
                                 C.c_void_p, C.c_size_t, C.c_void_p]),
    "ipsx_aggregate_packed": (C.c_int, [C.POINTER(Transf), C.c_void_p, C.c_void_p, C.c_void_p, C.c_int, C.c_int, C.c_void_p,
                                        C.c_void_p, C.c_size_t, C.c_void_p]),
    "ipsx_head": (C.c_int, [C.c_void_p, C.c_int, C.c_int, C.c_int, C.c_int, C.c_void_p, C.c_void_p,
                            C.c_int, C.c_int, C.c_void_p, C.c_void_p]),
    "ipsx_bn_train_supported": (C.c_int, [C.c_int64, C.c_int]),
    "ipsx_bn_train_workspace_floats": (C.c_size_t, [C.c_int64, C.c_int]),
    "ipsx_bn_train_forward": (C.c_int, [C.c_void_p, C.c_void_p, C.c_int64, C.c_int, C.c_void_p, C.c_void_p,
                                        C.c_float, C.c_float, C.c_void_p, C.c_void_p, C.c_int,
                                        C.c_void_p, C.c_void_p, C.c_void_p, C.c_void_p, C.c_void_p]),
    "ipsx_bn_train_backward": (C.c_int, [C.c_void_p, C.c_void_p, C.c_void_p, C.c_int64, C.c_int, C.c_void_p,
                                         C.c_void_p, C.c_void_p, C.c_int, C.c_void_p, C.c_void_p, C.c_void_p,
                                         C.c_void_p, C.c_void_p, C.c_void_p]),
    "ipsx_projector_train_supported": (C.c_int, [C.c_int, C.c_int]),
    "ipsx_projector_train_slabs": (C.c_int64, [C.c_int64]),
    "ipsx_projector_train_forward": (C.c_int, [C.POINTER(Conv), C.c_void_p, C.c_void_p, C.c_int, C.c_int64, C.c_void_p, C.c_void_p,
                                               C.c_void_p, C.c_void_p, C.c_void_p]),
    "ipsx_projector_wgrad_chunk_rows": (C.c_int64, []),
    "ipsx_projector_wgrad_max_rows": (C.c_int64, [C.c_int, C.c_int, C.c_int]),
    "ipsx_projector_wgrad_workspace_bytes": (C.c_size_t, [C.c_int64, C.c_int, C.c_int]),
    "ipsx_projector_wgrad": (C.c_int, [C.c_void_p, C.c_int, C.c_void_p, C.c_void_p, C.c_int64, C.c_int, C.c_int, C.c_void_p,
                                       C.c_void_p, C.c_int, C.c_void_p, C.c_size_t, C.c_void_p]),
    "ipsx_attn_pool_supported": (C.c_int, [C.c_int, C.c_int]),
    "ipsx_attn_pool_workspace_bytes": (C.c_size_t, [C.c_int64, C.c_int64, C.c_int, C.c_int]),
    "ipsx_attn_pool_forward": (C.c_int, [C.c_void_p, C.c_void_p, C.c_void_p, C.c_int64, C.c_int64, C.c_int, C.c_int, C.c_void_p,
                                         C.c_void_p, C.c_void_p, C.c_size_t, C.c_void_p]),
    "ipsx_attn_pool_backward": (C.c_int, [C.c_void_p, C.c_void_p, C.c_void_p, C.c_void_p, C.c_void_p, C.c_void_p, C.c_int64,
                                          C.c_int64, C.c_int, C.c_int, C.c_void_p, C.c_void_p, C.c_void_p, C.c_size_t, C.c_void_p]),
}


def library_path():
    return _SO


def build(verbose=False):
    cmd = ["make", "-C", os.path.join(_PKG, "csrc")] + ([] if verbose else ["-s"])
    subprocess.check_call(cmd)
    return _SO


def lib():
    global _LIB
    if _LIB is None:
        if not os.path.exists(_SO):
            raise RuntimeError(
                "libipsx.so not found at {} - build it with `python -c 'import __graft_entry__ as g; "
                "g.build()'` or `make -C ips_amd/csrc`; the HIP backend has no fallback".format(_SO))
        L = C.CDLL(_SO)
        for name, (res, args) in _EXPORTS.items():
            fn = getattr(L, name)
            fn.restype, fn.argtypes = res, args
        if L.ipsx_version() // 100 != ABI_MAJOR:
            raise RuntimeError("libipsx.so ABI version {} != {}.x (include/ipsx.h: the major number changes with every "
                               "incompatible change of an exported signature)".format(L.ipsx_version(), ABI_MAJOR))
        L.ipsx_set_tie_order(_TIE_MODES[tie_order()])
        if os.environ.get("IPSX_CAM_HEAD"):
            L.ipsx_dbg_stream_head.restype, L.ipsx_dbg_stream_head.argtypes = None, [C.c_int]
            L.ipsx_dbg_stream_head(int(os.environ["IPSX_CAM_HEAD"]))
        if os.environ.get("IPSX_SCAN_R8", "1") == "0":
            L.ipsx_dbg_scan_r8.argtypes = [C.c_int]
            L.ipsx_dbg_scan_r8(0)
        _LIB = L
    return _LIB


def _ck(rc, what):
    if rc != 0:
        raise RuntimeError("{} failed ({}): {}".format(what, rc, lib().ipsx_last_error().decode()))


def _stream():
    return C.c_void_p(_raw_stream(_cur_device()))


_raw_stream = getattr(torch._C, "_cuda_getCurrentRawStream", None)
_cur_device = getattr(torch._C, "_cuda_getDevice", None)
if _raw_stream is None or _cur_device is None:
    def _stream():
        return C.c_void_p(torch.cuda.current_stream().cuda_stream)


def _p(t):
    return C.c_void_p(t.data_ptr()) if t is not None else C.c_void_p(0)


def _f32(t):
    if t.dtype != torch.float32:
        raise TypeError("expected float32, got {}".format(t.dtype))
    return t if t.is_contiguous() else t.contiguous()


def _same_gpu(what, names, *tensors):
    dev = None
    for t in tensors:
        if t is not None:
            d = t.device
            if dev is None:
                if not _gpu_device(d):
                    raise ValueError("{}: {} lies on {}, the kernels read and write GPU memory".format(
                        what, [n for n, u in zip(names, tensors) if u is t][0], d))
                dev = d
            elif d != dev:
                raise ValueError("{}: {} lies on {}, the call's other tensors on {}".format(
                    what, [n for n, u in zip(names, tensors) if u is t][0], d, dev))
    return dev


def _one_gpu(what, **tensors):
    return _same_gpu(what, tuple(tensors), *tensors.values())


def _rd(what, name, t, dtype=torch.float32, dim=None, align=16, cl=False):
    if t.dtype != dtype:
        raise TypeError("{}: {} must be {}, got {}".format(what, name, dtype, t.dtype))
    if dim is not None and t.dim() != dim:
        raise ValueError("{}: {} must have {} dimensions, got {}".format(what, name, dim, tuple(t.shape)))
    if cl:
        if not t.is_contiguous(memory_format=torch.channels_last):
            return t.contiguous(memory_format=torch.channels_last)
    elif not t.is_contiguous():
        return t.contiguous()
    return t.clone() if t.data_ptr() % align else t


def _wr(what, name, t, dtype, shape=None, align=1, cl=False):
    if t.dtype != dtype or (shape is not None and tuple(t.shape) != tuple(shape)) or t.data_ptr() % align or \
            not (t.is_contiguous(memory_format=torch.channels_last) if cl else t.is_contiguous()):
        raise ValueError("{}: {} must be a {}{} {} tensor{}, got {} {} with strides {} at an address {} mod 16".format(
            what, name, "channels-last" if cl else "contiguous", " " + str(tuple(shape)) if shape is not None else "", dtype,
            " at a {}-byte address".format(align) if align > 1 else "", t.dtype, tuple(t.shape), t.stride(), t.data_ptr() % 16))
    return t


def _workspace(what, ws):
    return _wr(what, "workspace", ws, torch.uint8, align=16) if ws is not None else None


_PATCH_DTYPES = {torch.float32: 0, torch.bfloat16: 1, torch.float16: 2}


def _patch_table(table, n_chan, device):
    from .quant import check_table
    check_table(table, n_chan)
    if table.device != device:
# ... 141 lines not shown
def _word(what, name, t, n=1):
    if t.dtype != torch.int32 or t.numel() != n or not t.is_contiguous():
        raise ValueError("{}: {} must hold {} contiguous int32 word(s), got {} {}".format(what, name, n, t.dtype, tuple(t.shape)))
    return t


def part_wait(done, want, status, bit=1):
    _same_gpu("part_wait", ("done", "status"), done, status)
    _word("part_wait", "done", done)
    _word("part_wait", "status", status)
    _ck(lib().ipsx_part_wait(_p(done), int(want), _p(status), int(bit), _stream()), "ipsx_part_wait")


def logits_stats(emb, pos, vq, R, out, stats_x, stats_out, ln_eps):
    _same_gpu("logits_stats", ("emb", "stats_x", "stats_out"), emb, stats_x, stats_out)
    if vq.dtype != torch.float32:
        raise TypeError("logits_stats: vq must be the float32 folded query, got {}".format(vq.dtype))
    if out is None:
        raise ValueError("logits_stats: out must be given")
    stats_x = _rd("logits_stats", "stats_x", stats_x, dim=2)
    sn, sf = stats_x.shape
    _wr("logits_stats", "stats_out", stats_out, torch.float32, (sn, 2), align=8)
    emb, pos, pos_bs, out = _logits_args("logits_stats", emb, pos, vq, R, out, None)
    B, n, D = emb.shape
    _ck(lib().ipsx_logits_stats(_p(emb), n * D, _p(pos), pos_bs, _p(vq), B, n, D, R, _p(out), out.stride(0),
                                _p(stats_x), sn, sf, C.c_float(ln_eps), _p(stats_out), _stream()), "ipsx_logits_stats")
    return out


def scan_workspace(B, M, I, H, T, device):
    nb = lib().ipsx_scan_workspace_bytes(B, M, I, H, T)
    return torch.empty(nb, dtype=torch.uint8, device=device) if nb else None


def scan_workgroups_per_image(B, M, I, H, T):
    return max(1, int(lib().ipsx_scan_workgroups_per_image(B, M, I, H, T)))


def _scan_args(what, lg, M, I, H, T, mem_idx=None, tie=None, workspace=None, copy=True, words=()):
    _same_gpu(what, _SCAN_NAMES, lg, mem_idx, tie, workspace, *words)
    shape = lg.shape
    if len(shape) != 3 or shape[2] != H * T:
        raise ValueError("{}: lg must be (B, N, H*T = {}), got {}".format(what, H * T, tuple(shape)))
    B, N = shape[0], shape[1]
    if N <= M:
        raise ValueError("{}: lg has N = {} rows per image, the loop needs more than M = {}".format(what, N, M))
    if lg.dtype != torch.float32:
        raise TypeError("{}: lg must be float32, got {}".format(what, lg.dtype))
    if not lg.is_contiguous() or lg.data_ptr() & 15:
        if not copy:
            raise ValueError("{}: lg must be the whole contiguous (B, N, H*T) table at a 16-byte address (it is read where it "
                             "lies), got strides {}".format(what, lg.stride()))
        lg = lg.clone() if lg.is_contiguous() else lg.contiguous()
    if mem_idx is not None and (mem_idx.dtype != torch.int64 or mem_idx.shape != (B, M) or not mem_idx.is_contiguous()):
        raise ValueError("{}: mem_idx must be a contiguous ({}, {}) int64 tensor, got {} {}".format(what, B, M, mem_idx.dtype, tuple(mem_idx.shape)))
    if tie is not None and (tie.dtype != torch.int32 or tie.shape != (B,) or not tie.is_contiguous()):
        raise ValueError("{}: tie must be a contiguous ({},) int32 tensor, got {} {}".format(what, B, tie.dtype, tuple(tie.shape)))
    if workspace is not None:
        _workspace(what, workspace)
    return lg, B, N


_SCAN_NAMES = ("lg", "mem_idx", "tie", "workspace", "cond / ready", "status")


def scan(lg, M, I, H, T, want_scores=False):
    lg, B, N = _scan_args("scan", lg, M, I, H, T)
    mem_idx = torch.empty((B, M), dtype=torch.int64, device=lg.device)
    sc = torch.empty((B, M), dtype=torch.float32, device=lg.device) if want_scores else None
    tie = torch.zeros((B,), dtype=torch.int32, device=lg.device)
    ws = scan_workspace(B, M, I, H, T, lg.device)
    _ck(lib().ipsx_scan(_p(lg), B, N, M, I, H, T, _p(mem_idx), _p(sc), _p(tie), _p(ws), ws.numel() if ws is not None else 0,
                        _stream()), "ipsx_scan")
    scan.last_tie = tie
    return (mem_idx, sc) if want_scores else mem_idx


def scan_range(lg, M, I, H, T, it_begin, it_end, mem_idx, tie, workspace=None):
    lg, B, N = _scan_args("scan_range", lg, M, I, H, T, mem_idx, tie, workspace)
    ws = workspace if workspace is not None else scan_workspace(B, M, I, H, T, lg.device)
    _ck(lib().ipsx_scan_range(_p(lg), B, N, M, I, H, T, it_begin, it_end, _p(mem_idx), None, _p(tie),
                              _p(ws), ws.numel() if ws is not None else 0, _stream()), "ipsx_scan_range")
    return mem_idx


def scan_range_strided(lg, n, M, I, H, T, it_begin, it_end, mem_idx, tie, workspace=None):
    B, cap = lg.shape[:2]
    if lg.dtype != torch.float32 or lg.dim() != 3 or lg.stride(2) != 1 or lg.stride(1) != lg.shape[2] or (B > 1 and lg.stride(0) != cap * lg.shape[2]):
        raise ValueError("scan_range_strided needs a row-contiguous float32 (B, cap, H*T) logits table")
    if lg.shape[2] != H * T or lg.data_ptr() % 16:
        raise ValueError("scan_range_strided: lg must have H*T = {} columns and lie at a 16-byte address, got {}".format(H * T, tuple(lg.shape)))
    if not 0 < n <= cap:
        raise ValueError("{} candidates in a table of {} rows".format(n, cap))
    _one_gpu("scan_range_strided", lg=lg, mem_idx=mem_idx, tie=tie, workspace=workspace)
    _wr("scan_range_strided", "mem_idx", mem_idx, torch.int64, (B, M))
    _wr("scan_range_strided", "tie", tie, torch.int32, (B,))
    _workspace("scan_range_strided", workspace)
    ws = workspace if workspace is not None else scan_workspace(B, M, I, H, T, lg.device)
    _ck(lib().ipsx_scan_range_strided(_p(lg), cap, B, n, M, I, H, T, it_begin, it_end, _p(mem_idx), None, _p(tie),
                                      _p(ws), ws.numel() if ws is not None else 0, _stream()), "ipsx_scan_range_strided")
    return mem_idx


def scan_ragged(lg, offsets, lengths, M, I, H, T, want_scores=False, workspace=None, short_ok=False):
    lengths = [int(n) for n in lengths]
    B, total = len(lengths), sum(lengths)
    if B == 0:
        raise ValueError("scan_ragged: no slides")
    _one_gpu("scan_ragged", lg=lg, offsets=offsets, workspace=workspace)
    _workspace("scan_ragged", workspace)
    if lg.data_ptr() % 16:
        raise ValueError("scan_ragged: lg must lie at a 16-byte address")
    if lg.dtype != torch.float32 or lg.dim() != 2 or not lg.is_contiguous() or lg.shape != (total, H * T):
        raise ValueError("scan_ragged needs a contiguous float32 ({}, {}) logits table, got {} {}".format(
            total, H * T, lg.dtype, tuple(lg.shape)))
    if offsets.dtype != torch.int64 or tuple(offsets.shape) != (B + 1,) or not offsets.is_contiguous() or offsets.device != lg.device:
        raise ValueError("scan_ragged needs the ({},) int64 row offsets on the logits' device".format(B + 1))
    for k, n in enumerate(lengths):
        if n <= M and not short_ok:
            raise ValueError("slide {} has {} rows: the loop needs more than M = {}".format(k, n, M))
    if max(lengths) <= M:
        raise ValueError("scan_ragged: no slide has more than M = {} rows".format(M))
    mem_idx = torch.empty((B, M), dtype=torch.int64, device=lg.device)
    sc = torch.empty((B, M), dtype=torch.float32, device=lg.device) if want_scores else None
    tie = torch.empty((B,), dtype=torch.int32, device=lg.device)
    ws = workspace
    if ws is None:
        nb = lib().ipsx_scan_workspace_bytes(1, M, I, H, T)
        ws = torch.empty(B * nb, dtype=torch.uint8, device=lg.device) if nb else None
    _ck(lib().ipsx_scan_ragged(_p(lg), _p(offsets), B, max(lengths), total, M, I, H, T, _p(mem_idx), _p(sc), _p(tie), _p(ws),
                               ws.numel() if ws is not None else 0, _stream()), "ipsx_scan_ragged")
    scan_ragged.last_tie = tie
    return (mem_idx, sc) if want_scores else mem_idx


def _on_gpu(what, *tensors):
    dev = None
    for t in tensors:
        if t is None:
            continue
        if not _gpu_device(t.device) or (dev is not None and t.device != dev):
            raise ValueError("{}: every tensor lies on the GPU, all on the same one (got one on {})".format(what, t.device))
        dev = t.device


def scan_ragged_spans(lg, spans, n_max, M, I, H, T, mem_idx, tie, mem_score=None, workspace=None):
    _on_gpu("scan_ragged_spans", lg, spans, mem_idx, tie, mem_score, workspace)
    if lg.dtype != torch.float32 or lg.dim() != 2 or not lg.is_contiguous() or lg.shape[1] != H * T or lg.data_ptr() % 16:
        raise ValueError("scan_ragged_spans needs a contiguous float32 (rows, {}) logits table at a 16-byte address, got {} {}".format(
            H * T, lg.dtype, tuple(lg.shape)))
    _workspace("scan_ragged_spans", workspace)
    B = spans.shape[0] if spans.dim() == 2 else 0
    if spans.dtype != torch.int64 or tuple(spans.shape) != (B, 2) or B == 0 or not spans.is_contiguous() or spans.device != lg.device:
        raise ValueError("scan_ragged_spans needs (B, 2) int64 spans on the logits' device")
    if mem_idx.dtype != torch.int64 or tuple(mem_idx.shape) != (B, M) or not mem_idx.is_contiguous():
        raise ValueError("mem_idx must be a contiguous ({}, {}) int64 tensor".format(B, M))
    if tie.dtype != torch.int32 or tuple(tie.shape) != (B,) or not tie.is_contiguous():
        raise ValueError("tie must be a contiguous ({},) int32 tensor".format(B))
    if mem_score is not None and (mem_score.dtype != torch.float32 or tuple(mem_score.shape) != (B, M) or not mem_score.is_contiguous()):
        raise ValueError("mem_score must be a contiguous ({}, {}) float32 tensor".format(B, M))
    ws = workspace
    if ws is None:
        nb = lib().ipsx_scan_workspace_bytes(1, M, I, H, T)
        ws = torch.empty(B * nb, dtype=torch.uint8, device=lg.device) if nb else None
    _ck(lib().ipsx_scan_ragged_spans(_p(lg), _p(spans), B, int(n_max), lg.shape[0], M, I, H, T, _p(mem_idx), _p(mem_score), _p(tie),
                                     _p(ws), ws.numel() if ws is not None else 0, _stream()), "ipsx_scan_ragged_spans")
# ... 206 lines not shown

_PERSIST_CALLS = 0
_PERSIST_RECENT = []


def persistent_timed_out(dev):
    global _PERSIST_STRIKES
    import warnings
    _PERSIST_STRIKES += 1
    limit = max(1, int(os.environ.get("IPSX_PERSIST_STRIKES", "3") or 3))
    window = max(1, int(os.environ.get("IPSX_PERSIST_WINDOW", "1000") or 1000))
    _PERSIST_RECENT[:] = [c for c in _PERSIST_RECENT if _PERSIST_CALLS - c < window] + [_PERSIST_CALLS]
    what = "a persistent selection loop timed out waiting for rows (its call was redone with per-part launches: results valid)"
    if len(_PERSIST_RECENT) >= limit:
        persistent_disable("%s - %d such events within %d calls" % (what, len(_PERSIST_RECENT), window))
        return False
    dev = torch.device(dev)
    idx = dev.index if dev.index is not None else torch.cuda.current_device()
    ok = _PERSIST_OK[idx] = _persistent_selftest(torch.device("cuda", idx))
    if not ok:
        persistent_disable(what + "; a loop beside its producer no longer passes the device's self-test")
        return False
    warnings.warn("ips_amd: %s; the device's self-test passes, the persistent pipelines stay on (event %d of %d allowed within "
                  "%d calls; IPSX_PERSIST_WAIT_MS raises the wait, IPSX_PERSIST_STRIKES the allowance)"
                  % (what, len(_PERSIST_RECENT), limit, window))
    return True


def _persistent_selftest(dev):
    M = I = 16
    H, T = 8, 1
    if not scan_persistent_supported(M, I, H, T):
        return False
    N = M + 4 * I
    with torch.cuda.device(dev):
        lg = torch.zeros((1, N, H * T), dtype=torch.float32, device=dev)
        mem = torch.empty((1, M), dtype=torch.int64, device=dev)
        words = torch.zeros((3,), dtype=torch.int32, device=dev)
        side, main = side_stream(dev), torch.cuda.current_stream(dev)
        side.wait_stream(main)
        with torch.cuda.stream(side):
            scan_persistent(lg, M, I, H, T, mem, words[0:1], words[1:2], words[2:3])
        scan_gate(words[2:3])
        publish_rows(words[1:2], N)
        main.wait_stream(side)
        torch.cuda.synchronize(dev)
        status = int(words[2].item())
    return (status & 1) == 0 and (status & 2) == 2


_SIDE_STREAMS = {}


def side_stream(dev):
    dev = torch.device(dev)
    key = (dev.type, dev.index if dev.index is not None else torch.cuda.current_device())
    st = _SIDE_STREAMS.get(key)
    if st is None:
        st = _SIDE_STREAMS[key] = torch.cuda.Stream(device=dev, priority=-1)
    return st


def scan_persistent_supported(M, I, H, T):
    return bool(lib().ipsx_scan_persistent_supported(M, I, H, T))


def scan_persistent_large(M, I, H, T):
    return (not scan_persistent_supported(M, I, H, T) and lib().ipsx_scan_workspace_bytes(1, M, I, H, T) > 0
            and M + I <= 16384 and H * T <= 256)


def scan_mnist_shape(M, I, H, T):
    fn = lib().ipsx_dbg_scan_mnist_shape
    fn.restype, fn.argtypes = C.c_int, [C.c_int] * 4
    return bool(fn(M, I, H, T))


def dbg_scan_mnist(on):
    fn = lib().ipsx_dbg_scan_mnist
    fn.restype, fn.argtypes = None, [C.c_int]
    fn(1 if on else 0)


def scan_persistent_groupable(M, I, H, T):
    return bool(lib().ipsx_scan_persistent_groupable(M, I, H, T))


def scan_persistent(lg, M, I, H, T, mem_idx, tie, ready, status, workgroups=0, workspace=None, stream=None):
    lg, B, N = _scan_args("scan_persistent", lg, M, I, H, T, mem_idx, tie, workspace, False, (ready, status))
    _wr("scan_persistent", "ready", ready, torch.int32)
    if ready.numel() not in (1, B):
        raise ValueError("ready: one word, or one per image")
    _word("scan_persistent", "status", status)
    st = C.c_void_p(stream.cuda_stream) if stream is not None else _stream()
    if workspace is not None:
        _ck(lib().ipsx_scan_persistent_ws(_p(lg), B, N, M, I, H, T, _p(mem_idx), None, _p(tie), _p(ready),
                                          1 if (ready.numel() == B and B > 1) else 0, _p(status), int(workgroups),
                                          _p(workspace), workspace.numel(), st), "ipsx_scan_persistent_ws")
        return mem_idx
    _ck(lib().ipsx_scan_persistent_on(_p(lg), B, N, M, I, H, T, _p(mem_idx), None, _p(tie), _p(ready),
                                      1 if (ready.numel() == B and B > 1) else 0, _p(status), int(workgroups), st),
        "ipsx_scan_persistent_on")
    return mem_idx


def scan_gate(status):
    _same_gpu("scan_gate", ("status",), status)
    _word("scan_gate", "status", status)
    _ck(lib().ipsx_scan_gate(_p(status), _stream()), "ipsx_scan_gate")


def publish_rows(ready, n_rows):
    _same_gpu("publish_rows", ("ready",), ready)
    _word("publish_rows", "ready", ready)
    _ck(lib().ipsx_publish_rows(_p(ready), int(n_rows), _stream()), "ipsx_publish_rows")


def _scores_impl(x, qs, wk, H, Dk, T, want_attn):
    what = "attn_map" if want_attn else "scores"
    _one_gpu(what, x=x, qs=qs, wk=wk)
    x = _rd(what, "x", x, dim=3)
    B, L, D = x.shape
    qs, Dw = _fold_args(what, qs, wk, H, Dk, T)
    if Dw != D:
        raise ValueError("{}: x has {} features, wk takes {}".format(what, D, Dw))
    sc = torch.empty((B, L), dtype=torch.float32, device=x.device)
    attn = torch.empty((B, H, T, L), dtype=torch.float32, device=x.device) if want_attn else None
    nb = lib().ipsx_scores_workspace_bytes(B, L, D, H, T)
    ws = torch.empty(max(nb, 1), dtype=torch.uint8, device=x.device)
    wkp = pack_linear(wk)
    _ck(lib().ipsx_scores(_p(x), _p(wkp), _p(qs), B, L, D, H, Dk, T, _p(sc), _p(attn),
                          _p(ws), nb, _stream()), "ipsx_scores")
    return sc, attn


def scores(x, qs, wk, H, Dk, T):
    return _scores_impl(x, qs, wk, H, Dk, T, False)[0]


def attn_map(x, qs, wk, H, Dk, T):
    return _scores_impl(x, qs, wk, H, Dk, T, True)[1]


def topm(sc, M):
    _one_gpu("topm", sc=sc)
    sc = _rd("topm", "sc", sc, dim=2, align=4)
    B, L = sc.shape
    if not 0 < M <= L:
        raise ValueError("topm: M = {} of L = {} candidates".format(M, L))
    top = torch.empty((B, M), dtype=torch.int64, device=sc.device)
    tie = torch.zeros((B,), dtype=torch.int32, device=sc.device)
    nb = lib().ipsx_topm_workspace_bytes(B, L, M)
    ws = torch.empty(nb, dtype=torch.uint8, device=sc.device) if nb else None
    _ck(lib().ipsx_topm(_p(sc), B, L, M, _p(top), _p(tie), _p(ws), nb, _stream()), "ipsx_topm")
    return top


def gather_rows(src, idx):
    _same_gpu("gather_rows", ("src", "idx"), src, idx)
    if idx.dtype != torch.int64 or idx.dim() != 2:
        raise TypeError("gather_rows: idx must be a (B, M) int64 tensor, got {} {}".format(idx.dtype, tuple(idx.shape)))
    B, M = idx.shape
    if src.dim() < 2 or src.shape[0] not in (1, B):
        raise ValueError("gather_rows: src must be ({} or 1, N, ...) for idx {}, got {}".format(B, tuple(idx.shape), tuple(src.shape)))
    if src.stride(0) == 0 and src.shape[0] > 1:
        src = src[:1]
# ... 463 lines not shown
```

### ips_amd/selection.py

```python

import contextlib
import ctypes as C
import gc
import math
import os
import weakref

import torch

from . import hip


@contextlib.contextmanager
def _no_gc_pause():
    was = gc.isenabled()
    if was:
        gc.disable()
    try:
        yield
    finally:
        if was:
            gc.enable()


def _env_on(name):
    return os.environ.get(name, "1") != "0"


NATIVE_ORDER_DEFAULT = "0"

ONE_LAUNCH_U8_DEFAULT = "0"


def _native_order_on():
    return os.environ.get("IPSX_NATIVE_ORDER", NATIVE_ORDER_DEFAULT) == "1"


class Selection:

    OVERLAP_PARTS = 4
    LAZY_SLAB_BYTES = 48 << 20

    def __init__(self, net, owned=False):
        self._net = weakref.ref(net) if owned else (lambda: net)
        self._bufs = {}
        self._side = None
        self._copy = None
        self.scan_status = None
        self.scan_status_host = None
        self._mirror_pending = None
        self._unfinished = None
        self._done = None
        self._calls = {}
        self.timing_hook = None
        self._part_index = None
        self._order = None
        self._order_bn = None
        self._flat_made = None
        self._flat_key = None
        self._flat_base = None
        self._part_map = None
        self._one_piece_index = {}
        self.index_calls = 0
        self.view_calls = 0
        self.native_calls = 0
        self.native_ordered_calls = 0

    @property
    def net(self):
        return self._net()

    def plan(self):
        return self.net.plan

    @property
    def _flat(self):
        if self._order is None:
            return None
        if self._flat_made is None:
            self._flat_made = self.flat_index(self._order, *self._order_bn)
        return self._flat_made

    def status_mirror(self):
        if self.scan_status_host is None:
            self.scan_status_host = torch.zeros((1,), dtype=torch.int32).pin_memory()
        return self.scan_status_host

    def check_strike(self, dev):
        mirror = self.scan_status_host
        if mirror is not None and int(mirror.item()) & 1:
            mirror.zero_()
            hip.persistent_timed_out(dev)

    def n_iter(self, N):
        return math.ceil((N - self.net.M) / self.net.I)

    def streams(self, dev):
        if self._side is None or self._side.device != torch.device(dev):
            self._side = hip.side_stream(dev)
        return self._side, torch.cuda.current_stream(dev)

    def buffers(self, name, key, make):
        held = self._bufs.get(name)
        if held is None or held[0] != key:
            bufs = make()
            side = self._side
            for t in bufs:
                if t is not None and side is not None:
                    t.record_stream(side)
            self._bufs[name] = held = (key, bufs)
        return held[1]

    def persistent_allowed(self, dev, M, I, H, T, loops=1, large=False):
        return (_env_on("IPSX_SCAN_PERSIST") and _env_on("IPSX_OVERLAP_SCAN") and not hip.dedup_blank()
                and (hip.scan_persistent_supported(M, I, H, T) or (large and hip.scan_persistent_large(M, I, H, T)))
                and hip.device_geometry(dev).cus >= 8 * max(1, loops)
                and hip.persistent_ok(dev))

    def persistent_begin(self, logits, mem_idx_buf, zeroed, B, dev, loops=0, scan_ws=None, zero_words=None):
        (zeroed if zero_words is None else zeroed[:zero_words]).zero_()
        hip._PERSIST_CALLS += 1
        net = self.net
        ca = net.transf.crs_attn
        self.check_strike(dev)
        side, main = self.streams(dev)
        tie, words, ctl = zeroed[:B], zeroed[B:2 * B + 1], zeroed[2 * B + 1:]
        ready, status = words[:B], words[B:B + 1]
        self.scan_status = status
        side.wait_stream(main)
        hip.scan_persistent(logits, net.M, net.I, ca.H, ca.n_token, mem_idx_buf, tie, ready, status, workgroups=loops,
                            workspace=scan_ws, stream=side)
        hip.scan_gate(status)
        return tie, ready, status, ctl

# ... 338 lines not shown
                            hip.publish_rows(ready[b_:b_ + 1], rows)
        net._emb_parts = [emb_buf]
        return self.persistent_end(logits, mem_idx_buf, tie, status, n_iter, dev, scan_ws)

    def image_stream(self, patches, pos_enc):
        net, plan = self.net, self.plan()
        N = patches.shape[1]
        M, I, dev = net.M, net.I, patches.device
        ca = net.transf.crs_attn
        vq, R = ca.folded_query(), ca.H * ca.n_token
        self.streams(dev)
        logits, mem_idx_buf, emb_buf, zeroed = self.buffers(
            "image", (N, M, I, R, net.D, str(dev)),
            lambda: (torch.empty((1, N, R), dtype=torch.float32, device=dev),
                     torch.empty((1, M), dtype=torch.int64, device=dev),
                     torch.empty((1, N, net.D), dtype=torch.float32, device=dev),
                     torch.zeros((3 + plan.image_stream_ctl_words(N),), dtype=torch.int32, device=dev)))
        ordered = self._order is not None
        if patches.dtype == torch.float32 and self.native_ok(patches, pos_enc if net.use_pos else None):
            tp = (pos_enc[0] if pos_enc[0].is_contiguous() else pos_enc[0].contiguous()) if net.use_pos else None
            return self.native_call("image", patches, pos_enc if net.use_pos else None, logits, mem_idx_buf, zeroed, emb_buf, None, 0, 0,
                                    trunk_pos=tp, quad_pulls=-1)
        fidx = self._flat.view(-1) if ordered else None
        with _no_gc_pause():
            tie, ready, status, ctl = self.persistent_begin(logits, mem_idx_buf, zeroed, 1, dev)
            plan.image_stream(patches[0], pos_enc[0] if net.use_pos else None, vq, R, emb_buf[0], logits[0], ctl, ready,
                              index=fidx)
        net._emb_parts = [emb_buf]
        return self.persistent_end(logits, mem_idx_buf, tie, status, self.n_iter(N), dev)

    @staticmethod
    def part_lists(B, N, edges, dev):
        rows = torch.arange(B, device=dev, dtype=torch.int32).unsqueeze(1) * N
        return [(rows + torch.arange(edges[k], edges[k + 1], device=dev, dtype=torch.int32)).reshape(-1)
                for k in range(len(edges) - 1)]

    @staticmethod
    def part_map(B, N, edges, dev):
        pos = torch.arange(B * N, device=dev).view(B, N)
        return torch.cat([pos[:, edges[k]:edges[k + 1]].reshape(-1) for k in range(len(edges) - 1)])

    @staticmethod
    def part_ends(B, edges):
        return [B * e for e in edges[1:]]

    def one_launch_ok(self, src, fused, small, vq, P):
        if src is not None and src.dtype == torch.uint8 and os.environ.get("IPSX_ONE_LAUNCH_U8", ONE_LAUNCH_U8_DEFAULT) == "0":
            return False
        return (src is not None and fused and not small and 2 <= P <= 16 and src.dtype in (torch.float32, torch.uint8)
                and hip.precision() == "fp32"
                and vq.dtype == torch.float32 and src.count < (1 << 31) - 16
                and _env_on("IPSX_ONE_LAUNCH") and hip.persistent_ok(src.device))

    @staticmethod
    def one_launch_dedup(src):
        return (hip.dedup_auto() and src.dtype in (torch.float32, torch.uint8)
                and (src.table is not None) == (src.dtype == torch.uint8))

    def parts_one_launch(self, src, every, edges, its, pos_enc, vq, R):
        net, plan = self.net, self.plan()
        N = edges[-1]
        B = every.numel() // N
        M, I, dev = net.M, net.I, src.device
        ca = net.transf.crs_attn
        P = len(its) - 1
        hip._PERSIST_CALLS += 1
        self.check_strike(dev)
        side, main = self.streams(dev)
        logits, mem_idx_buf, words, scan_ws = self.buffers(
            "parts1", (B, N, M, I, R, P, str(dev)),
            lambda: (torch.empty((B, N, R), dtype=torch.float32, device=dev),
                     torch.empty((B, M), dtype=torch.int64, device=dev),
                     torch.zeros((-(-(B + P + 1) // 4) * 4,), dtype=torch.int32, device=dev),
                     hip.scan_workspace(B, M, I, ca.H, ca.n_token, dev)))
        tie, done, status = words[:B], words[B:B + P], words[B + P:B + P + 1]
        words.zero_()
        zeroed = torch.cuda.Event()
        zeroed.record(main)
        ends = self.part_ends(B, edges)
        emb_all = plan.encode_source(src, index=every, parts=(ends, done), dedup=self.one_launch_dedup(src))
        emb_all.record_stream(side)
        starts = [0] + ends[:-1]
        net._emb_parts = parts = [emb_all[starts[k]:ends[k]].view(B, edges[k + 1] - edges[k], -1) for k in range(P)]
        pos = [pos_enc[:, edges[k]:edges[k + 1]] if net.use_pos else None for k in range(P)]
        with torch.cuda.stream(side):
            side.wait_event(zeroed)
            for k in range(P - 1):
                hip.part_wait(done[k:k + 1], ends[k] - starts[k], status)
                hip.logits(parts[k], pos[k], vq, R, out=logits[:, edges[k]:edges[k + 1]])
                hip.scan_range(logits, M, I, ca.H, ca.n_token, its[k], its[k + 1], mem_idx_buf, tie, scan_ws)
        main.wait_stream(side)
        k = P - 1
        hip.logits(parts[k], pos[k], vq, R, out=logits[:, edges[k]:edges[k + 1]])
        hip.scan_range(logits, M, I, ca.H, ca.n_token, its[k], its[k + 1], mem_idx_buf, tie, scan_ws)
        for k in range(P - 1):
            hip.logits(parts[k], pos[k], vq, R, out=logits[:, edges[k]:edges[k + 1]], cond=status)
        hip.scan_range_if(logits, M, I, ca.H, ca.n_token, 0, its[P], mem_idx_buf, tie, status, 1, workspace=scan_ws)
        self._mirror_pending = status
        hip.scan.last_tie = tie
        return mem_idx_buf.clone()

    def parts_with_ranges(self, patches, pos_enc):
        net, plan = self.net, self.plan()
        B, N = patches.shape[:2]
        M, I, dev = net.M, net.I, patches.device
        ca = net.transf.crs_attn
        vq, R = ca.folded_query(), ca.H * ca.n_token
        n_iter = self.n_iter(N)
        from .dist import part_iterations
        src = self.source(patches)
        fused = src is not None and bool(plan.fused(src.shape))
        indexed = fused or (src is not None and src.is_view)
        edges, small = None, False
        if net.is_image and B * N < self.small_batch_limit(dev) and n_iter < 100:
            edges, its = self.small_batch_split(B, N, dev)
            small = True
        elif net.is_image and indexed and hip.precision() == "bf16":
            from .dist import launch_model, plan_iterations
            its = plan_iterations(N, M, I, 1, B, launch_model(net, tuple(patches.shape[2:]), hip.device_geometry(dev).cus),
                                  self.OVERLAP_PARTS)
        elif net.is_image:
            its = part_iterations(n_iter, self.OVERLAP_PARTS)
        else:
            its = self.feature_parts(B, N, dev, False)
        P = len(its) - 1
        if edges is None:
            edges = [0] + [min(N, M + it * I) for it in its[1:]]
            edges[-1] = N
        key = (B, N, tuple(edges), str(dev))
        if indexed and (self._part_index is None or self._part_index[0] != key):
            lists = self.part_lists(B, N, edges, dev)
            self._part_index = (key, lists, torch.cat(lists))
        side, main = self.streams(dev)
        flat = patches.reshape(B * N, *patches.shape[2:]) if self._flat is not None and not indexed else None
        part_index = self._part_index[1] if indexed else None
        every = self._part_index[2] if indexed else None
        if self._flat is not None:
            if self._part_map is None or self._part_map[0] != key:
                self._part_map = (key, self.part_map(B, N, edges, dev))
            every = torch.index_select(self._flat.reshape(-1), 0, self._part_map[1])
            part_index = [every[B * edges[k]:B * edges[k + 1]] for k in range(P)]
        if self.one_launch_ok(src, fused, small, vq, P):
            return self.parts_one_launch(src, every, edges, its, pos_enc, vq, R)
        logits, mem_idx_buf, tie, scan_ws = self.buffers(
            "parts", (B, N, M, I, R, str(dev)),
            lambda: (torch.empty((B, N, R), dtype=torch.float32, device=dev),
                     torch.empty((B, M), dtype=torch.int64, device=dev),
                     torch.zeros((B,), dtype=torch.int32, device=dev),
                     hip.scan_workspace(B, M, I, ca.H, ca.n_token, dev)))
        tie.zero_()
        net._emb_parts = parts = []
        side.wait_stream(main)
        for k in range(P):
            lo, hi = edges[k], edges[k + 1]
            if indexed:
                emb = plan.encode_source(src, index=part_index[k]).view(B, hi - lo, -1)
            elif self._flat is not None:
                emb = plan.encode(flat, index=part_index[k]).view(B, hi - lo, -1)
            else:
                emb = net._embed(patches[:, lo:hi].reshape(-1, *patches.shape[2:])).view(B, hi - lo, -1)
            parts.append(emb)
            pos = pos_enc[:, lo:hi] if net.use_pos else None
            if k == P - 1:
                main.wait_stream(side)
                hip.logits(emb, pos, vq, R, out=logits[:, lo:hi])
                hip.scan_range(logits, M, I, ca.H, ca.n_token, its[k], its[k + 1], mem_idx_buf, tie, scan_ws)
                continue
            done = torch.cuda.Event()
            done.record(main)
            emb.record_stream(side)
            with torch.cuda.stream(side):
                side.wait_event(done)
                hip.logits(emb, pos, vq, R, out=logits[:, lo:hi])
                hip.scan_range(logits, M, I, ca.H, ca.n_token, its[k], its[k + 1], mem_idx_buf, tie, scan_ws)
        main.wait_stream(side)
        hip.scan.last_tie = tie
        return mem_idx_buf.clone()

    def slabs(self, patches, pos_enc):
        net = self.net
        B, N = patches.shape[:2]
        M, I, dev = net.M, net.I, net.device
        ca = net.transf.crs_attn
# ... 107 lines not shown
```

Measured before the change: 38.02 million patches/s.

## Fuse logits computation into MNIST scan kernel prologue for overlapped parts

Moves the logits MFMA wave routine into a shared header and adds a prologue variant of the MNIST scan kernel. Each workgroup computes logits for its image's parts before scanning, which removes the separate logits launch per part and the conditional redo launches. A redo flag makes the last call recompute all parts if any earlier part was skipped. The clone of the memory index is also skipped when the caller finishes the selection. Parts larger than a row limit keep the separate logits kernel. The risk is that one workgroup per image computes logits serially, which limits parallelism for large parts.

```diff
diff --git a/include/ipsx.h b/include/ipsx.h
--- a/include/ipsx.h
+++ b/include/ipsx.h
@@ -293,6 +293,17 @@
 int ipsx_scan_range_if(const float* logits, int b, int64_t n, int m, int i, int h, int n_token,
                        int64_t it_begin, int64_t it_end, int64_t* mem_idx, float* mem_score,
                        int32_t* tie_flag, const int32_t* cond, int32_t cond_mask, void* stream);
+typedef struct ipsx_logits_part {
+    const float* emb;
+    int64_t rows;
+    int64_t first;
+} ipsx_logits_part;
+int ipsx_scan_logits_check(const ipsx_logits_part* parts, int n_parts, int part_begin, int part_end, int64_t n, int m, int i,
+                           int64_t it_begin, int64_t it_end);
+int ipsx_scan_range_logits(float* logits, int b, int64_t n, int m, int i, int h, int n_token, int64_t it_begin, int64_t it_end,
+                           int64_t* mem_idx, float* mem_score, int32_t* tie_flag, const ipsx_logits_part* parts, int n_parts,
+                           int part_begin, int part_end, int d, const float* pos, int64_t pos_bstride, const float* v_packed,
+                           const int32_t* redo, int32_t redo_mask, void* stream);
 int ipsx_logits_stats(const float* emb, int64_t emb_bstride, const float* pos, int64_t pos_bstride,
                       const float* v_packed, int b, int64_t n, int d, int r, float* logits, int64_t logits_bstride,
                       const float* stats_x, int64_t stats_n, int stats_f, float ln_eps, float* stats_out, void* stream);
diff --git a/ips_amd/architecture/ips_net.py b/ips_amd/architecture/ips_net.py
--- a/ips_amd/architecture/ips_net.py
+++ b/ips_amd/architecture/ips_net.py
@@ -262,7 +262,11 @@
 
             if hip.on_device(device):
                 with self.plan.hold():
-                    mem_idx = self._select_hip(patches, pos_enc, order)
+                    self.selection.caller_finishes = True
+                    try:
+                        mem_idx = self._select_hip(patches, pos_enc, order)
+                    finally:
+                        self.selection.caller_finishes = False
             else:
                 mem_idx = self._select_aten(patches, pos_enc)
 
diff --git a/ips_amd/csrc/logits.hip b/ips_amd/csrc/logits.hip
--- a/ips_amd/csrc/logits.hip
+++ b/ips_amd/csrc/logits.hip
@@ -2,6 +2,7 @@
 #include <algorithm>
 #include <cstdlib>
 
+#include "logits_wave.h"
 #include "scan_common.h"
 
 namespace ipsx {
@@ -34,117 +35,6 @@
         }
     }
     vp[(((size_t)(r >> 5) * kgs + (c >> 3)) * 64 + (r & 31) + 32 * ((c & 7) >> 2)) * 4 + (c & 3)] = acc;
-}
-
-struct LogitsArgs {
-    const float* emb; long long emb_bs;
-    const float* pos; long long pos_bs;
-    const float* vp;
-    long long n;
-    int d, R, kgs;
-    float* out; long long out_bs;
-};
-
-template <int NT>
-__device__ __forceinline__ void logits_wave(const LogitsArgs& a, unsigned bx, int bi) {
-    const int lane = threadIdx.x & 63, wave = threadIdx.x >> 6, half = lane >> 5;
-    const long long r0 = ((long long)bx * 4 + wave) * 32;
-    if (r0 >= a.n) return;
-    const long long row = r0 + (lane & 31);
-    const bool rv = row < a.n;
-    const float* e = a.emb + (size_t)bi * a.emb_bs + (size_t)(rv ? row : 0) * a.d + 4 * half;
-    const float* p = a.pos ? a.pos + (size_t)bi * a.pos_bs + (size_t)(rv ? row : 0) * a.d + 4 * half : nullptr;
-
-    f32x16 acc[NT];
-#pragma unroll
-    for (int i = 0; i < NT; ++i)
-#pragma unroll
-        for (int r = 0; r < 16; ++r) acc[i][r] = 0.0f;
-
-    const float4* vq = reinterpret_cast<const float4*>(a.vp) + lane;
-    const bool vec = (a.d & 7) == 0;
-    int kg0 = 0;
-    if (vec) {
-        float4 ev[2][8], bv[2][NT][8];
-        auto fetch = [&](int k0, int set) {
-#pragma unroll
-            for (int u = 0; u < 8; ++u) {
-                ev[set][u] = *reinterpret_cast<const float4*>(e + (k0 + u) * 8);
-                if (p) {
-                    const float4 pv = *reinterpret_cast<const float4*>(p + (k0 + u) * 8);
-                    ev[set][u].x = ev[set][u].x + pv.x; ev[set][u].y = ev[set][u].y + pv.y;
-                    ev[set][u].z = ev[set][u].z + pv.z; ev[set][u].w = ev[set][u].w + pv.w;
-                }
-#pragma unroll
-                for (int i = 0; i < NT; ++i) bv[set][i][u] = vq[((size_t)i * a.kgs + k0 + u) * 64];
-            }
-        };
-        auto mma = [&](int set) {
-#pragma unroll
-            for (int u = 0; u < 8; ++u) {
-                const float a0 = rv ? ev[set][u].x : 0.0f, a1 = rv ? ev[set][u].y : 0.0f;
-                const float a2 = rv ? ev[set][u].z : 0.0f, a3 = rv ? ev[set][u].w : 0.0f;
-#pragma unroll
-                for (int i = 0; i < NT; ++i) {
-                    acc[i] = __builtin_amdgcn_mfma_f32_32x32x2f32(a0, bv[set][i][u].x, acc[i], 0, 0, 0);
-                    acc[i] = __builtin_amdgcn_mfma_f32_32x32x2f32(a1, bv[set][i][u].y, acc[i], 0, 0, 0);
-                    acc[i] = __builtin_amdgcn_mfma_f32_32x32x2f32(a2, bv[set][i][u].z, acc[i], 0, 0, 0);
-                    acc[i] = __builtin_amdgcn_mfma_f32_32x32x2f32(a3, bv[set][i][u].w, acc[i], 0, 0, 0);
-                }
-            }
-        };
-        if (a.kgs >= 8) {
-            fetch(0, 0);
-            for (; kg0 + 16 <= a.kgs; kg0 += 16) {
-                fetch(kg0 + 8, 1);
-                mma(0);
-                if (kg0 + 24 <= a.kgs) fetch(kg0 + 16, 0);
-                mma(1);
-            }
-            if (kg0 + 8 <= a.kgs) { mma(0); kg0 += 8; }
-        }
-    }
-    for (int kg = kg0; kg < a.kgs; ++kg) {
-        float av[4];
-        if (vec) {
-            const float4 ev = *reinterpret_cast<const float4*>(e + kg * 8);
-            av[0] = ev.x; av[1] = ev.y; av[2] = ev.z; av[3] = ev.w;
-            if (p) {
-                const float4 pv = *reinterpret_cast<const float4*>(p + kg * 8);
-                av[0] = av[0] + pv.x; av[1] = av[1] + pv.y; av[2] = av[2] + pv.z; av[3] = av[3] + pv.w;
-            }
-#pragma unroll
-            for (int j = 0; j < 4; ++j) av[j] = rv ? av[j] : 0.0f;
-        } else {
-#pragma unroll
-            for (int j = 0; j < 4; ++j) {
-                const int c = kg * 8 + j;
-                float v = (c + 4 * half < a.d) ? e[c] : 0.0f;
-                if (p) v = v + ((c + 4 * half < a.d) ? p[c] : 0.0f);
-                av[j] = rv ? v : 0.0f;
-            }
-        }
-#pragma unroll
-        for (int i = 0; i < NT; ++i) {
-            const float4 b = vq[((size_t)i * a.kgs + kg) * 64];
-            acc[i] = __builtin_amdgcn_mfma_f32_32x32x2f32(av[0], b.x, acc[i], 0, 0, 0);
-            acc[i] = __builtin_amdgcn_mfma_f32_32x32x2f32(av[1], b.y, acc[i], 0, 0, 0);
-            acc[i] = __builtin_amdgcn_mfma_f32_32x32x2f32(av[2], b.z, acc[i], 0, 0, 0);
-            acc[i] = __builtin_amdgcn_mfma_f32_32x32x2f32(av[3], b.w, acc[i], 0, 0, 0);
-        }
-    }
-    float* out = a.out + (size_t)bi * a.out_bs;
-#pragma unroll
-    for (int i = 0; i < NT; ++i) {
-        const int o = i * 32 + (lane & 31);
-        if (o < a.R) {
-#pragma unroll
-            for (int r = 0; r < 16; ++r) {
-                const long long rr = r0 + (r & 3) + 8 * (r >> 2) + 4 * half;
-                if (rr < a.n) out[(size_t)rr * a.R + o] = acc[i][r];
-            }
-        }
-    }
 }
 
 template <int NT>
diff --git a/ips_amd/csrc/logits_wave.h b/ips_amd/csrc/logits_wave.h
--- /dev/null
+++ b/ips_amd/csrc/logits_wave.h
@@ -0,0 +1,118 @@
+#pragma once
+
+#include "scan_common.h"
+
+namespace ipsx {
+
+struct LogitsArgs {
+    const float* emb; long long emb_bs;
+    const float* pos; long long pos_bs;
+    const float* vp;
+    long long n;
+    int d, R, kgs;
+    float* out; long long out_bs;
+};
+
+template <int NT, int U = 8, int WAVES = 4, int POS = 0>
+__device__ __forceinline__ void logits_wave(const LogitsArgs& a, unsigned bx, int bi) {
+    const int lane = threadIdx.x & 63, wave = threadIdx.x >> 6, half = lane >> 5;
+    const long long r0 = ((long long)bx * WAVES + wave) * 32;
+    if (r0 >= a.n) return;
+    const long long row = r0 + (lane & 31);
+    const bool rv = row < a.n;
+    const float* e = a.emb + (size_t)bi * a.emb_bs + (size_t)(rv ? row : 0) * a.d + 4 * half;
+    const float* p = a.pos ? a.pos + (size_t)bi * a.pos_bs + (size_t)(rv ? row : 0) * a.d + 4 * half : nullptr;
+
+    f32x16 acc[NT];
+#pragma unroll
+    for (int i = 0; i < NT; ++i)
+#pragma unroll
+        for (int r = 0; r < 16; ++r) acc[i][r] = 0.0f;
+
+    const float4* vq = reinterpret_cast<const float4*>(a.vp) + lane;
+    const bool vec = (a.d & 7) == 0;
+    int kg0 = 0;
+    if (vec) {
+        float4 ev[2][U], bv[2][NT][U];
+        auto fetch = [&](int k0, int set) {
+#pragma unroll
+            for (int u = 0; u < U; ++u) {
+                ev[set][u] = *reinterpret_cast<const float4*>(e + (k0 + u) * 8);
+                if (POS == 0 ? p != nullptr : POS > 0) {
+                    const float4 pv = *reinterpret_cast<const float4*>(p + (k0 + u) * 8);
+                    ev[set][u].x = ev[set][u].x + pv.x; ev[set][u].y = ev[set][u].y + pv.y;
+                    ev[set][u].z = ev[set][u].z + pv.z; ev[set][u].w = ev[set][u].w + pv.w;
+                }
+#pragma unroll
+                for (int i = 0; i < NT; ++i) bv[set][i][u] = vq[((size_t)i * a.kgs + k0 + u) * 64];
+            }
+        };
+        auto mma = [&](int set) {
+#pragma unroll
+            for (int u = 0; u < U; ++u) {
+                const float a0 = rv ? ev[set][u].x : 0.0f, a1 = rv ? ev[set][u].y : 0.0f;
+                const float a2 = rv ? ev[set][u].z : 0.0f, a3 = rv ? ev[set][u].w : 0.0f;
+#pragma unroll
+                for (int i = 0; i < NT; ++i) {
+                    acc[i] = __builtin_amdgcn_mfma_f32_32x32x2f32(a0, bv[set][i][u].x, acc[i], 0, 0, 0);
+                    acc[i] = __builtin_amdgcn_mfma_f32_32x32x2f32(a1, bv[set][i][u].y, acc[i], 0, 0, 0);
+                    acc[i] = __builtin_amdgcn_mfma_f32_32x32x2f32(a2, bv[set][i][u].z, acc[i], 0, 0, 0);
+                    acc[i] = __builtin_amdgcn_mfma_f32_32x32x2f32(a3, bv[set][i][u].w, acc[i], 0, 0, 0);
+                }
+            }
+        };
+        if (a.kgs >= U) {
+            fetch(0, 0);
+            for (; kg0 + 2 * U <= a.kgs; kg0 += 2 * U) {
+                fetch(kg0 + U, 1);
+                mma(0);
+                if (kg0 + 3 * U <= a.kgs) fetch(kg0 + 2 * U, 0);
+                mma(1);
+            }
+            if (kg0 + U <= a.kgs) { mma(0); kg0 += U; }
+        }
+    }
+    for (int kg = kg0; kg < a.kgs; ++kg) {
+        float av[4];
+        if (vec) {
+            const float4 ev = *reinterpret_cast<const float4*>(e + kg * 8);
+            av[0] = ev.x; av[1] = ev.y; av[2] = ev.z; av[3] = ev.w;
+            if (p) {
+                const float4 pv = *reinterpret_cast<const float4*>(p + kg * 8);
+                av[0] = av[0] + pv.x; av[1] = av[1] + pv.y; av[2] = av[2] + pv.z; av[3] = av[3] + pv.w;
+            }
+#pragma unroll
+            for (int j = 0; j < 4; ++j) av[j] = rv ? av[j] : 0.0f;
+        } else {
+#pragma unroll
+            for (int j = 0; j < 4; ++j) {
+                const int c = kg * 8 + j;
+                float v = (c + 4 * half < a.d) ? e[c] : 0.0f;
+                if (p) v = v + ((c + 4 * half < a.d) ? p[c] : 0.0f);
+                av[j] = rv ? v : 0.0f;
+            }
+        }
+#pragma unroll
+        for (int i = 0; i < NT; ++i) {
+            const float4 b = vq[((size_t)i * a.kgs + kg) * 64];
+            acc[i] = __builtin_amdgcn_mfma_f32_32x32x2f32(av[0], b.x, acc[i], 0, 0, 0);
+            acc[i] = __builtin_amdgcn_mfma_f32_32x32x2f32(av[1], b.y, acc[i], 0, 0, 0);
+            acc[i] = __builtin_amdgcn_mfma_f32_32x32x2f32(av[2], b.z, acc[i], 0, 0, 0);
+            acc[i] = __builtin_amdgcn_mfma_f32_32x32x2f32(av[3], b.w, acc[i], 0, 0, 0);
+        }
+    }
+    float* out = a.out + (size_t)bi * a.out_bs;
+#pragma unroll
+    for (int i = 0; i < NT; ++i) {
+        const int o = i * 32 + (lane & 31);
+        if (o < a.R) {
+#pragma unroll
+            for (int r = 0; r < 16; ++r) {
+                const long long rr = r0 + (r & 3) + 8 * (r >> 2) + 4 * half;
+                if (rr < a.n) out[(size_t)rr * a.R + o] = acc[i][r];
+            }
+        }
+    }
+}
+
+}
diff --git a/ips_amd/csrc/scan_common.h b/ips_amd/csrc/scan_common.h
--- a/ips_amd/csrc/scan_common.h
+++ b/ips_amd/csrc/scan_common.h
@@ -928,6 +928,17 @@
     int64_t table_rows = 0;
 };
 
+constexpr int SCAN_LOGITS_PARTS = 16;
+struct LogitsPart { const float* emb; int rows, first; };
+struct ScanLogits {
+    LogitsPart part[SCAN_LOGITS_PARTS];
+    const float* pos; long long pos_bs;
+    const float* vp;
+    float* out;
+    const int* redo; int redo_mask;
+    int d, kgs, n_parts, part0, part1;
+};
+
 inline const long long* slide_entries(const ScanCall& c) {
     static_assert(sizeof(long long) == sizeof(int64_t), "slide tables: 64-bit entries");
     return static_cast<const long long*>(static_cast<const void*>(c.slide_table));
@@ -944,6 +955,7 @@
 int launch_scan_cam(const ScanCall& c);
 bool scan_mnist_shape(int m, int i, int h, int n_token);
 int launch_scan_mnist(const ScanCall& c);
+int launch_scan_mnist_logits(const ScanCall& c, const ScanLogits& p);
 size_t scan_large_ws_per_image(int m, int i, int h, int n_token);
 int launch_scan_large(const ScanCall& c);
 int scan_large_team(int b, int m, int i, int h, int n_token);
@@ -959,6 +971,7 @@
 extern int g_scan_team;
 extern bool g_scan_r8;
 extern bool g_scan_mnist;
+extern bool g_scan_logits;
 extern unsigned long long* g_scan_stamps;
 unsigned long long* persist_log();
 
diff --git a/ips_amd/csrc/scan_mnist.hip b/ips_amd/csrc/scan_mnist.hip
--- a/ips_amd/csrc/scan_mnist.hip
+++ b/ips_amd/csrc/scan_mnist.hip
@@ -2,6 +2,7 @@
 #include <algorithm>
 #include <cstdlib>
 
+#include "logits_wave.h"
 #include "scan_common.h"
 
 namespace ipsx {
@@ -30,11 +31,34 @@
     return as_float((uint32_t)__builtin_amdgcn_update_dpp(0, (int)as_u32(v), K * 0x55, 0xF, 0xF, false));
 }
 
-template <bool PERSIST>
-__global__ __launch_bounds__(mn::NT) void scan_mnist_kernel(ScanArgs a) {
+template <bool PRO, bool PERSIST, typename... P>
+__global__ __launch_bounds__(mn::NT) void scan_mnist_kernel(ScanArgs a, P... p) {
     using namespace mn;
+    static_assert(sizeof...(P) == (PRO ? 1 : 0) && !(PRO && PERSIST), "scan_mnist_kernel: the prologue's arguments, plain launches only");
     extern __shared__ __attribute__((aligned(16))) unsigned char smem[];
     if (!PERSIST && scan_skipped(a.cond, a.cond_mask)) return;
+    if constexpr (PRO) {
+        const ScanLogits& q = (p, ...);
+        int k0 = q.part0, k1 = q.part1;
+        int redo = 0;
+        if (q.redo != nullptr)
+            redo = __builtin_amdgcn_readfirstlane(__hip_atomic_load(q.redo, __ATOMIC_RELAXED, __HIP_MEMORY_SCOPE_AGENT) & q.redo_mask);
+        if (redo != 0) { k0 = 0; k1 = q.n_parts; a.it0 = 0; }
+#pragma unroll 1
+        for (int k = k0; k < k1; ++k) {
+            LogitsArgs la;
+            la.emb = q.part[k].emb; la.emb_bs = (long long)q.part[k].rows * q.d;
+            la.pos = q.pos ? q.pos + (size_t)q.part[k].first * q.d : nullptr; la.pos_bs = q.pos_bs;
+            la.vp = q.vp; la.n = q.part[k].rows; la.d = q.d; la.R = R; la.kgs = q.kgs;
+            la.out = q.out + (size_t)q.part[k].first * R; la.out_bs = a.n * R;
+            if (q.pos) {
+                for (unsigned bx = 0; (long long)bx * (NT / 2) < la.n; ++bx) logits_wave<1, 4, NT / 64, 1>(la, bx, (int)blockIdx.x);
+            } else {
+                for (unsigned bx = 0; (long long)bx * (NT / 2) < la.n; ++bx) logits_wave<1, 4, NT / 64, -1>(la, bx, (int)blockIdx.x);
+            }
+        }
+        __builtin_amdgcn_fence(__ATOMIC_RELEASE, "workgroup");
+    }
     __builtin_amdgcn_s_setprio(3);
     if (PERSIST) {
         asm volatile("v_mov_b32 v127, 0" ::: "v127");
@@ -58,6 +82,7 @@
     if (tid < 4 * R) pmax[tid] = 0u;
     if (tid < 2) ccount[2 + tid] = 0;
     lds_barrier();
+    if constexpr (PRO) __builtin_amdgcn_fence(__ATOMIC_ACQUIRE, "workgroup");
     SCAN_WAIT_ROWS(std::min<long long>(a.n, a.it0 * (long long)I + M + I));
     {
         float* const x0 = reinterpret_cast<float*>(smem + OFF_X);
@@ -286,8 +311,19 @@
     ScanArgs a;
     fill_scan_args(a, c);
     a.stk_off = mn::OFF_STK;
-    launch_lds(c.ready ? scan_mnist_kernel<true> : scan_mnist_kernel<false>, dim3((unsigned)c.b), dim3(mn::NT), mn::LDS_BYTES, c.stream, a);
+    launch_lds(c.ready ? scan_mnist_kernel<false, true> : scan_mnist_kernel<false, false>, dim3((unsigned)c.b), dim3(mn::NT), mn::LDS_BYTES,
+               c.stream, a);
     return launched("scan");
 }
 
-}
+int launch_scan_mnist_logits(const ScanCall& c, const ScanLogits& p) {
+    IPSX_REQUIRE(scan_mnist_shape(c.m, c.i, c.h, c.n_token) && c.rows == Rows::Packed && !c.ready && !c.cond && c.workgroups <= 0,
+                 "scan_mnist_kernel with logits: 8 heads x 4 tokens, M = I = 64, packed logits, a plain launch of one workgroup per image");
+    ScanArgs a;
+    fill_scan_args(a, c);
+    a.stk_off = mn::OFF_STK;
+    launch_lds(scan_mnist_kernel<true, false, ScanLogits>, dim3((unsigned)c.b), dim3(mn::NT), mn::LDS_BYTES, c.stream, a, p);
+    return launched("scan_logits");
+}
+
+}
diff --git a/ips_amd/csrc/scorer.hip b/ips_amd/csrc/scorer.hip
--- a/ips_amd/csrc/scorer.hip
+++ b/ips_amd/csrc/scorer.hip
@@ -15,6 +15,7 @@
 bool g_scan_direct = true;
 bool g_scan_r8 = true;
 bool g_scan_mnist = true;
+bool g_scan_logits = true;
 unsigned long long* g_scan_stamps = nullptr;
 
 __device__ unsigned long long g_persist_log[8];
@@ -282,6 +283,66 @@
     return dispatch_scan(c);
 }
 
+IPSX_API int ipsx_scan_logits_check(const ipsx_logits_part* parts, int n_parts, int part_begin, int part_end, int64_t n, int m,
+                                    int i, int64_t it_begin, int64_t it_end) {
+    IPSX_REQUIRE(parts && n_parts >= 1 && n_parts <= SCAN_LOGITS_PARTS, "scan_range_logits: 1 to %d parts (got %d)", SCAN_LOGITS_PARTS, n_parts);
+    IPSX_REQUIRE(part_begin >= 0 && part_begin <= part_end && part_end <= n_parts, "scan_range_logits: parts [%d, %d) of %d", part_begin,
+                 part_end, n_parts);
+    IPSX_REQUIRE(m > 0 && i > 0 && n > m && n < ((int64_t)1 << 31), "scan_range_logits: more patches (%lld, fewer than 2^31) than memory slots (%d)",
+                 (long long)n, m);
+    int64_t at = 0;
+    for (int k = 0; k < n_parts; ++k) {
+        IPSX_REQUIRE(parts[k].rows > 0 && parts[k].rows <= n, "scan_range_logits: part %d has %lld rows per image", k, (long long)parts[k].rows);
+        IPSX_REQUIRE(parts[k].first == at, "scan_range_logits: part %d starts at row %lld, the parts in front of it end at %lld", k,
+                     (long long)parts[k].first, (long long)at);
+        at += parts[k].rows;
+    }
+    IPSX_REQUIRE(at == n, "scan_range_logits: the parts hold %lld rows per image, an image has %lld", (long long)at, (long long)n);
+    IPSX_REQUIRE(it_begin >= 0 && it_begin < it_end && it_end <= (n - m + i - 1) / i, "scan_range_logits: iteration range [%lld, %lld) outside the loop",
+                 (long long)it_begin, (long long)it_end);
+    const int64_t read_end = std::min<int64_t>(n, (int64_t)m + it_end * i);
+    const int64_t have_end = part_end > 0 ? parts[part_end - 1].first + parts[part_end - 1].rows : 0;
+    IPSX_REQUIRE(read_end <= have_end, "scan_range_logits: iterations up to %lld read rows up to %lld, the parts in front of part %d end at %lld",
+                 (long long)it_end, (long long)read_end, part_end, (long long)have_end);
+    return IPSX_OK;
+}
+
+IPSX_API int ipsx_scan_range_logits(float* logits, int b, int64_t n, int m, int i, int h, int n_token, int64_t it_begin, int64_t it_end,
+                                    int64_t* mem_idx, float* mem_score, int32_t* tie_flag, const ipsx_logits_part* parts, int n_parts,
+                                    int part_begin, int part_end, int d, const float* pos, int64_t pos_bstride, const float* v_packed,
+                                    const int32_t* redo, int32_t redo_mask, void* stream) {
+    IPSX_REQUIRE(logits && mem_idx && v_packed && b > 0, "scan_range_logits: null pointer");
+    IPSX_REQUIRE(scan_mnist_shape(m, i, h, n_token), "scan_range_logits: 8 heads x 4 tokens, M = I = 64 (scan_mnist_kernel) only");
+    IPSX_REQUIRE(d > 0 && d % 8 == 0, "scan_range_logits: embeddings of whole 8-float groups (d = %d)", d);
+    IPSX_REQUIRE(!redo == !redo_mask, "scan_range_logits: the redo word and its mask go together");
+    IPSX_TRY(ipsx_scan_logits_check(parts, n_parts, part_begin, part_end, n, m, i, it_begin, it_end));
+    for (int k = 0; k < n_parts; ++k)
+        IPSX_REQUIRE(parts[k].emb && (reinterpret_cast<uintptr_t>(parts[k].emb) & 15) == 0, "scan_range_logits: part %d's embeddings at a 16-byte address", k);
+    IPSX_REQUIRE((reinterpret_cast<uintptr_t>(v_packed) & 15) == 0 && (reinterpret_cast<uintptr_t>(pos) & 15) == 0 && pos_bstride >= 0 &&
+                 pos_bstride % 4 == 0, "scan_range_logits: the folded query and the positional table at 16-byte addresses");
+    const int r = h * n_token;
+    if (!g_scan_logits) {
+        for (int k = part_begin; k < part_end; ++k)
+            IPSX_TRY(ipsx_logits(parts[k].emb, parts[k].rows * d, pos ? pos + parts[k].first * d : nullptr, pos_bstride, v_packed, b, parts[k].rows, d, r,
+                                 logits + parts[k].first * r, n * r, stream));
+        IPSX_TRY(ipsx_scan_range(logits, b, n, m, i, h, n_token, it_begin, it_end, mem_idx, mem_score, tie_flag, nullptr, 0, stream));
+        if (!redo) return IPSX_OK;
+        for (int k = 0; k < n_parts; ++k)
+            if (k < part_begin || k >= part_end)
+                IPSX_TRY(ipsx_logits_if(parts[k].emb, parts[k].rows * d, pos ? pos + parts[k].first * d : nullptr, pos_bstride, v_packed, b, parts[k].rows,
+                                        d, r, logits + parts[k].first * r, n * r, redo, redo_mask, stream));
+        return ipsx_scan_range_if(logits, b, n, m, i, h, n_token, 0, it_end, mem_idx, mem_score, tie_flag, redo, redo_mask, stream);
+    }
+    ScanCall c = scan_call(logits, b, n, m, i, h, n_token, mem_idx, mem_score, tie_flag, stream);
+    c.it_begin = it_begin; c.it_end = it_end;
+    IPSX_TRY(validate_scan_call(c));
+    ScanLogits p = {};
+    for (int k = 0; k < n_parts; ++k) { p.part[k].emb = parts[k].emb; p.part[k].rows = (int)parts[k].rows; p.part[k].first = (int)parts[k].first; }
+    p.pos = pos; p.pos_bs = pos_bstride; p.vp = v_packed; p.out = logits; p.redo = redo; p.redo_mask = redo_mask;
+    p.d = d; p.kgs = d / 8; p.n_parts = n_parts; p.part0 = part_begin; p.part1 = part_end;
+    return launch_scan_mnist_logits(c, p);
+}
+
 IPSX_API int ipsx_set_persistent_wait_ms(int ms) {
     const int prev = g_persist_wait_ms;
     if (ms > 0) g_persist_wait_ms = ms > 20000 ? 20000 : ms;
@@ -311,6 +372,11 @@
 extern "C" __attribute__((visibility("default"))) void ipsx_dbg_scan_team_trunc(int on) { g_scan_team_trunc = on != 0; }
 extern "C" __attribute__((visibility("default"))) void ipsx_dbg_scan_r8(int on) { g_scan_r8 = on != 0; }
 extern "C" __attribute__((visibility("default"))) void ipsx_dbg_scan_mnist(int on) { g_scan_mnist = on != 0; }
+extern "C" __attribute__((visibility("default"))) int ipsx_dbg_scan_logits(int on) {
+    const int prev = g_scan_logits ? 1 : 0;
+    if (on >= 0) g_scan_logits = on != 0;
+    return prev;
+}
 extern "C" __attribute__((visibility("default"))) int ipsx_dbg_scan_mnist_shape(int m, int i, int h, int n_token) {
     return scan_mnist_shape(m, i, h, n_token) ? 1 : 0;
 }
diff --git a/ips_amd/hip.py b/ips_amd/hip.py
--- a/ips_amd/hip.py
+++ b/ips_amd/hip.py
@@ -329,6 +329,10 @@
                                                         C.c_void_p, C.c_int64, C.c_void_p, C.POINTER(C.c_int64), C.c_int, C.c_void_p,
                                                         C.c_void_p, C.c_void_p, C.c_size_t, C.c_void_p, C.c_void_p]),
     "ipsx_part_wait": (C.c_int, [C.c_void_p, C.c_int32, C.c_void_p, C.c_int32, C.c_void_p]),
+    "ipsx_scan_logits_check": (C.c_int, [C.c_void_p, C.c_int, C.c_int, C.c_int, C.c_int64, C.c_int, C.c_int, C.c_int64, C.c_int64]),
+    "ipsx_scan_range_logits": (C.c_int, [C.c_void_p, C.c_int, C.c_int64, C.c_int, C.c_int, C.c_int, C.c_int, C.c_int64, C.c_int64,
+                                         C.c_void_p, C.c_void_p, C.c_void_p, C.c_void_p, C.c_int, C.c_int, C.c_int, C.c_int, C.c_void_p,
+                                         C.c_int64, C.c_void_p, C.c_void_p, C.c_int32, C.c_void_p]),
     "ipsx_logits_if": (C.c_int, [C.c_void_p, C.c_int64, C.c_void_p, C.c_int64, C.c_void_p, C.c_int, C.c_int64, C.c_int, C.c_int,
                                  C.c_void_p, C.c_int64, C.c_void_p, C.c_int32, C.c_void_p]),
     "ipsx_trunk_encode_u8": (C.c_int, [C.POINTER(Trunk), C.c_void_p, C.c_void_p, C.c_int64, C.c_void_p, C.c_void_p,
@@ -451,6 +455,9 @@
         if os.environ.get("IPSX_SCAN_R8", "1") == "0":
             L.ipsx_dbg_scan_r8.argtypes = [C.c_int]
             L.ipsx_dbg_scan_r8(0)
+        if os.environ.get("IPSX_SCAN_LOGITS", "1") == "0":
+            L.ipsx_dbg_scan_logits.restype, L.ipsx_dbg_scan_logits.argtypes = C.c_int, [C.c_int]
+            L.ipsx_dbg_scan_logits(0)
         _LIB = L
     return _LIB
 
@@ -758,6 +765,61 @@
     _ck(lib().ipsx_scan_range(_p(lg), B, N, M, I, H, T, it_begin, it_end, _p(mem_idx), None, _p(tie),
                               _p(ws), ws.numel() if ws is not None else 0, _stream()), "ipsx_scan_range")
     return mem_idx
+
+
+class LogitsPartStruct(C.Structure):
+    _fields_ = [("emb", C.c_void_p), ("rows", C.c_int64), ("first", C.c_int64)]
+
+
+class LogitsParts:
+
+    def __init__(self, embs=None, rows=None):
+        if embs is not None:
+            rows = [int(e.shape[1]) for e in embs]
+        self.embs, self.rows = embs, [int(r) for r in rows]
+        self.first = [sum(self.rows[:k]) for k in range(len(self.rows))]
+        self.n = sum(self.rows)
+        self.array = (LogitsPartStruct * max(1, len(self.rows)))()
+        for k, r in enumerate(self.rows):
+            self.array[k].emb = embs[k].data_ptr() if embs is not None else None
+            self.array[k].rows, self.array[k].first = r, self.first[k]
+
+    def __len__(self):
+        return len(self.rows)
+
+    def check(self, part_begin, part_end, M, I, it_begin, it_end):
+        _ck(lib().ipsx_scan_logits_check(self.array, len(self), part_begin, part_end, self.n, M, I, it_begin, it_end),
+            "ipsx_scan_logits_check")
+
+    def scan_range(self, logits, M, I, H, T, it_begin, it_end, mem_idx, tie, part_begin, part_end, pos, vq, redo=None, mask=1):
+        _same_gpu("scan_range_logits", ("logits", "mem_idx", "tie", "pos", "vq", "redo") + ("emb",) * len(self), logits, mem_idx, tie, pos, vq,
+                  redo, *self.embs)
+        lg, B, N = _scan_args("scan_range_logits", logits, M, I, H, T, mem_idx, tie, None, False)
+        D = self.embs[0].shape[2]
+        for k, e in enumerate(self.embs):
+            if e.dtype != torch.float32 or e.dim() != 3 or tuple(e.shape) != (B, self.rows[k], D) or not e.is_contiguous() or e.data_ptr() & 15:
+                raise ValueError("scan_range_logits: part {} must be a contiguous float32 ({}, {}, {}) block at a 16-byte address, got {} {}".format(
+                    k, B, self.rows[k], D, e.dtype, tuple(e.shape)))
+        if self.n != N:
+            raise ValueError("scan_range_logits: the parts hold {} rows per image, the logits table {}".format(self.n, N))
+        size = lib().ipsx_folded_query_elems(H * T, 1, D)
+        if vq.dtype != torch.float32 or vq.numel() != size or vq.data_ptr() & 15 or not vq.is_contiguous():
+            raise ValueError("scan_range_logits: vq must be the contiguous float32 folded query of R = {}, D = {} at a 16-byte address".format(H * T, D))
+        pos_bs = 0
+        if pos is not None:
+            ps, st = pos.shape, pos.stride()
+            if pos.dtype != torch.float32 or len(ps) != 3 or ps[1] < N or ps[2] != D or ps[0] not in (1, B):
+                raise ValueError("scan_range_logits: pos must be float32 ({} or 1, >= {}, {}), got {} {}".format(B, N, D, pos.dtype, tuple(ps)))
+            pos_bs = st[0] if ps[0] > 1 else 0
+            if st[2] != 1 or st[1] != D or pos_bs < 0 or pos.data_ptr() & 15 or pos_bs & 3:
+                pos = pos.contiguous()
+                pos_bs = pos.stride(0) if ps[0] > 1 else 0
+        if redo is not None:
+            _word("scan_range_logits", "redo", redo)
+        _ck(lib().ipsx_scan_range_logits(_p(lg), B, N, M, I, H, T, it_begin, it_end, _p(mem_idx), None, _p(tie), self.array, len(self),
+                                         part_begin, part_end, D, _p(pos), pos_bs, _p(vq), _p(redo), mask if redo is not None else 0,
+                                         _stream()), "ipsx_scan_range_logits")
+        return mem_idx
 
 
 def scan_range_strided(lg, n, M, I, H, T, it_begin, it_end, mem_idx, tie, workspace=None):
@@ -1130,6 +1192,16 @@
     fn(1 if on else 0)
 
 
+def dbg_scan_logits(on):
+    fn = lib().ipsx_dbg_scan_logits
+    fn.restype, fn.argtypes = C.c_int, [C.c_int]
+    return bool(fn(-1 if on is None else (1 if on else 0)))
+
+
+def scan_logits_on():
+    return dbg_scan_logits(None)
+
+
 def scan_persistent_groupable(M, I, H, T):
     return bool(lib().ipsx_scan_persistent_groupable(M, I, H, T))
 
diff --git a/ips_amd/selection.py b/ips_amd/selection.py
--- a/ips_amd/selection.py
+++ b/ips_amd/selection.py
@@ -29,6 +29,8 @@
 
 NATIVE_ORDER_DEFAULT = "0"
 
+SCAN_LOGITS_ROWS_DEFAULT = "128"
+
 ONE_LAUNCH_U8_DEFAULT = "0"
 
 
@@ -39,6 +41,7 @@
 class Selection:
 
     OVERLAP_PARTS = 4
+    SCAN_LOGITS_ROWS = int(os.environ.get("IPSX_SCAN_LOGITS_ROWS", SCAN_LOGITS_ROWS_DEFAULT))
     LAZY_SLAB_BYTES = 48 << 20
 
     def __init__(self, net, owned=False):
@@ -50,6 +53,7 @@
         self.scan_status_host = None
         self._mirror_pending = None
         self._unfinished = None
+        self.caller_finishes = False
         self._done = None
         self._calls = {}
         self.timing_hook = None
@@ -554,6 +558,9 @@
         emb_all.record_stream(side)
         starts = [0] + ends[:-1]
         net._emb_parts = parts = [emb_all[starts[k]:ends[k]].view(B, edges[k + 1] - edges[k], -1) for k in range(P)]
+        if self.scan_logits_ok(vq, M, I, ca, net.D):
+            return self.parts_loop_logits(src, parts, its, pos_enc if net.use_pos else None, vq, logits, mem_idx_buf, tie, done, status,
+                                          [ends[k] - starts[k] for k in range(P)], zeroed, scan_ws)
         pos = [pos_enc[:, edges[k]:edges[k + 1]] if net.use_pos else None for k in range(P)]
         with torch.cuda.stream(side):
             side.wait_event(zeroed)
@@ -571,6 +578,45 @@
         self._mirror_pending = status
         hip.scan.last_tie = tie
         return mem_idx_buf.clone()
+
+    @staticmethod
+    def scan_logits_ok(vq, M, I, ca, D):
+        return (vq.dtype == torch.float32 and D % 8 == 0 and hip.scan_mnist_shape(M, I, ca.H, ca.n_token) and hip.scan_logits_on())
+
+    def parts_loop_logits(self, src, parts, its, pos, vq, logits, mem_idx_buf, tie, done, status, counts, zeroed, scan_ws=None):
+        net = self.net
+        M, I = net.M, net.I
+        ca = net.transf.crs_attn
+        P = len(its) - 1
+        side, main = self.streams(logits.device)
+        table = hip.LogitsParts(parts)
+        limit = self.SCAN_LOGITS_ROWS
+        R = ca.H * ca.n_token
+
+        def part(k, redo=None):
+            if table.rows[k] <= limit:
+                table.scan_range(logits, M, I, ca.H, ca.n_token, its[k], its[k + 1], mem_idx_buf, tie, k, k + 1, pos, vq, redo=redo)
+                return
+            lo = table.first[k]
+            hip.logits(parts[k], pos[:, lo:lo + table.rows[k]] if pos is not None else None, vq, R, out=logits[:, lo:lo + table.rows[k]])
+            if redo is None:
+                hip.scan_range(logits, M, I, ca.H, ca.n_token, its[k], its[k + 1], mem_idx_buf, tie, scan_ws)
+            else:
+                table.scan_range(logits, M, I, ca.H, ca.n_token, its[k], its[k + 1], mem_idx_buf, tie, k + 1, k + 1, pos, vq, redo=redo)
+
+        with torch.cuda.stream(side):
+            side.wait_event(zeroed)
+            for k in range(P - 1):
+                hip.part_wait(done[k:k + 1], counts[k], status)
+                part(k)
+        main.wait_stream(side)
+        part(P - 1, redo=status)
+        self._mirror_pending = status
+        hip.scan.last_tie = tie
+        if src.is_view or not self.caller_finishes:
+            return mem_idx_buf.clone()
+        self._unfinished = mem_idx_buf
+        return mem_idx_buf
 
     def parts_with_ranges(self, patches, pos_enc):
         net, plan = self.net, self.plan()
```

Result: faster. 38.89 million patches/s, median of 6 (+2.3%).
